# glaretechnologies/substrata

Hardware: AMD Instinct MI355X
Metric: physics steps/sec at fixed dt, 100k bodies (higher is better)
Workload: dtype f32; 1 GPU; BASELINE config 3: 100000 mixed box/sphere/capsule bodies, 100x100x10 lattice spacing 1.5 m, seed 3, ground quad 2000 m, dt 1/60, Jolt default settings (10 velocity / 2 position iterations), sleeping enabled; bodies_per_gpu=100000, tiles=1, active_bodies_end=99193, contact_constraints_start=296641, contact_constraints_end=299690, contact_points_end=362045, colours_end=21, contact_constraints_after_settle=293058, dropped_pairs_or_manifolds=0

## Files before the change

### substrata_amd/csrc/sgp_dev_common.h

```cpp
#pragma once
#include "sgp_kernels.h"
#include <algorithm>
#include "sgp_device_collide.h"
#include "sgp_device_vehicle.h"
#include "sgp_device_mesh.h"

#define TPB 256


SGP_DEV const ConstraintArrays& CUR(const DV& d) { return d.ca[d.sp->parity & 1]; }
SGP_DEV const ConstraintArrays& PRV(const DV& d) { return d.ca[(d.sp->parity & 1) ^ 1]; }
SGP_DEV uint2 con_ab(const ConstraintArrays& c, size_t k) { return *(const uint2*)(c.hdr + k); }
SGP_DEV int& con_npc(const ConstraintArrays& c, size_t k) { return ((int*)(c.hdr + k))[2]; }
SGP_DEV uint4 con_hdr(const ConstraintArrays& c, size_t k) { return c.hdr[k]; }

SGP_DEV uint32_t f_motion(uint32_t f) { return f & BF_MOTION_MASK; }
SGP_DEV uint32_t f_layer(uint32_t f) { return (f & BF_LAYER_MASK) >> BF_LAYER_SHIFT; }
SGP_DEV uint32_t f_shape(uint32_t f) { return (f & BF_SHAPE_MASK) >> BF_SHAPE_SHIFT; }
SGP_DEV bool f_movable(uint32_t f) { return (f & (BF_ALIVE | BF_ACTIVE)) == (BF_ALIVE | BF_ACTIVE) && f_motion(f) == SGP_MOTION_DYNAMIC; }
SGP_DEV uint32_t xcd_block() { return (blockIdx.x & 7u) * (gridDim.x >> 3) + (blockIdx.x >> 3); }
SGP_DEV bool f_active_for_pairs(uint32_t f) { return (f & (BF_ALIVE | BF_ACTIVE)) == (BF_ALIVE | BF_ACTIVE) && f_motion(f) != SGP_MOTION_STATIC; }

SGP_DEV bool layers_collide(uint32_t l1, uint32_t l2)
{
	if (l1 == SGP_LAYER_NON_MOVING) return l2 == SGP_LAYER_MOVING;
	if (l1 == SGP_LAYER_MOVING) return l2 != SGP_LAYER_NON_MOVING_NON_COLLIDABLE && l2 != SGP_LAYER_MOVING_NON_COLLIDABLE;
	return false;
}

SGP_DEV const sgd_hull* body_hull(const DV& d, float4 sh) { return &d.hulls[(uint32_t)sh.x]; }

SGP_DEV v3 shape_local_half(const DV& d, uint32_t type, float4 sh)
{
	if (type == SGP_SHAPE_MESH) return V3(1.0f, 1.0f, 1.0f);
	if (type == SGP_SHAPE_HULL) {
		const sgd_hull* h = body_hull(d, sh);
		return V3(fmaxf(fabsf(h->aabb_min.x), fabsf(h->aabb_max.x)), fmaxf(fabsf(h->aabb_min.y), fabsf(h->aabb_max.y)), fmaxf(fabsf(h->aabb_min.z), fabsf(h->aabb_max.z)));
	}
	if (type == SGP_SHAPE_SPHERE) return V3(sh.x, sh.x, sh.x);
	if (type == SGP_SHAPE_BOX) return V3(sh.x, sh.y, sh.z);
	return V3(sh.x, sh.x, sh.y + sh.x);
}

SGP_DEV float shape_volume(const DV& d, uint32_t type, float4 sh)
{
	if (type == SGP_SHAPE_MESH) return 0.0f;
	if (type == SGP_SHAPE_HULL) return body_hull(d, sh)->volume;
	if (type == SGP_SHAPE_SPHERE) return (4.0f / 3.0f) * 3.14159265358979323846f * sh.x * sh.x * sh.x;
	if (type == SGP_SHAPE_BOX) return 8.0f * sh.x * sh.y * sh.z;
	return 3.14159265358979323846f * sh.x * sh.x * (2.0f * sh.y) + (4.0f / 3.0f) * 3.14159265358979323846f * sh.x * sh.x * sh.x;
}

SGP_DEV void compute_aabb(const DV& d, uint32_t type, float4 sh, v3 pos, quat q, v3& mn, v3& mx)
{
	v3 e;
	if (type == SGP_SHAPE_MESH) {
		const MeshHeader mh = d.meshes[(uint32_t)sh.x];
		const m33 R = quat_to_m33(q);
		v3 lo = V3(3.4e38f, 3.4e38f, 3.4e38f), hi = V3(-3.4e38f, -3.4e38f, -3.4e38f);
		for (int k = 0; k < 8; ++k) {
			const v3 c = V3((k & 1) ? mh.mxx : mh.mnx, (k & 2) ? mh.mxy : mh.mny, (k & 4) ? mh.mxz : mh.mnz);
			const v3 p = m33_mul(R, c);
			lo = V3(fminf(lo.x, p.x), fminf(lo.y, p.y), fminf(lo.z, p.z)); hi = V3(fmaxf(hi.x, p.x), fmaxf(hi.y, p.y), fmaxf(hi.z, p.z));
		}
		mn = v3_add(pos, lo); mx = v3_add(pos, hi);
		return;
	}
	if (type == SGP_SHAPE_HULL) {
		const sgd_hull* h = body_hull(d, sh);
		const m33 R = quat_to_m33(q);
		v3 lo = V3(3.4e38f, 3.4e38f, 3.4e38f), hi = V3(-3.4e38f, -3.4e38f, -3.4e38f);
		for (int i = 0; i < h->nv; ++i) {
			const v3 p = m33_mul(R, h->verts[i]);
			lo = V3(fminf(lo.x, p.x), fminf(lo.y, p.y), fminf(lo.z, p.z)); hi = V3(fmaxf(hi.x, p.x), fmaxf(hi.y, p.y), fmaxf(hi.z, p.z));
		}
		mn = v3_add(pos, lo); mx = v3_add(pos, hi);
		return;
	}
	if (type == SGP_SHAPE_SPHERE) e = V3(sh.x, sh.x, sh.x);
	else {
		const m33 R = quat_to_m33(q);
		if (type == SGP_SHAPE_BOX) {
			e = V3(fabsf(R.c0.x) * sh.x + fabsf(R.c1.x) * sh.y + fabsf(R.c2.x) * sh.z,
			       fabsf(R.c0.y) * sh.x + fabsf(R.c1.y) * sh.y + fabsf(R.c2.y) * sh.z,
			       fabsf(R.c0.z) * sh.x + fabsf(R.c1.z) * sh.y + fabsf(R.c2.z) * sh.z);
		} else {
			e = V3(fabsf(R.c2.x) * sh.y + sh.x, fabsf(R.c2.y) * sh.y + sh.x, fabsf(R.c2.z) * sh.y + sh.x);
		}
	}
	mn = v3_sub(pos, e);
	mx = v3_add(pos, e);
}

SGP_DEV void sleep_points(const DV& d, uint32_t type, float4 sh, v3 pos, quat q, v3 out[3])
{
	const v3 ext = shape_local_half(d, type, sh);
	const m33 R = quat_to_m33(q);
	int lowest = 0;
	if (ext.y < v3_get(ext, lowest)) lowest = 1;
	if (ext.z < v3_get(ext, lowest)) lowest = 2;
	const int i1 = lowest == 0 ? 1 : 0;
	const int i2 = lowest == 2 ? 1 : 2;
	out[0] = pos;
	out[1] = v3_add(pos, v3_scale(m33_col(R, i1), v3_get(ext, i1)));
	out[2] = v3_add(pos, v3_scale(m33_col(R, i2), v3_get(ext, i2)));
}

SGP_DEV void reset_sleep(const DV& d, uint32_t i, uint32_t type, float4 sh, v3 pos, quat q)
{
	v3 p[3];
	sleep_points(d, type, sh, pos, q, p);
	d.sleep_s[0][i] = F4(p[0], 0.0f);
	d.sleep_s[1][i] = F4(p[1], 0.0f);
	d.sleep_s[2][i] = F4(p[2], 0.0f);
	d.sleep_timer[i] = 0.0f;
}

SGP_DEV void push_event(uint32_t* list, uint32_t* counter, uint32_t cap, uint32_t id)
{
	const uint32_t k = atomicAdd(counter, 1u);
	if (k < cap) list[k] = id;
}

SGP_DEV void step_end_block(const DV& d, StepCounters* host_mapped, EventWindow* host_events)
{
	const uint32_t* src = (const uint32_t*)d.ctr;
	uint32_t* dst = (uint32_t*)host_mapped;
	for (uint32_t i = threadIdx.x; i < sizeof(StepCounters) / 4; i += blockDim.x) dst[i] = src[i];
	__syncthreads();
	if (threadIdx.x == 0 && d.ts_nt) { host_mapped->ts_error = d.ts_flags[0]; host_mapped->ts_all_adjacent = d.ts_flags[1]; }
	if (threadIdx.x < sizeof(EventCounters) / 4) ((uint32_t*)&host_events->c)[threadIdx.x] = ((const uint32_t*)d.evc)[threadIdx.x];
	const uint32_t win = min(min(d.ev_window, SGP_EVENT_WINDOW), d.cap_bodies);
	const uint32_t* lists[3] = { d.ev_activated, d.ev_deactivated, d.ev_water };
	const uint32_t counts[3] = { d.evc->n_activated, d.evc->n_deactivated, d.evc->n_water };
	for (int l = 0; l < 3; ++l) {
		if (counts[l] > win) continue;
		for (uint32_t i = threadIdx.x; i < counts[l]; i += blockDim.x) host_events->ids[l][i] = lists[l][i];
	}
}

SGP_DEV bool last_block(uint32_t* ticket)
{
	__shared__ uint32_t s_last_ticket;
	__syncthreads();
	if (threadIdx.x == 0) { __threadfence(); s_last_ticket = atomicAdd(ticket, 1u); }
	__syncthreads();
	const bool last = s_last_ticket == gridDim.x - 1u;
	if (last) __threadfence();
	return last;
}

SGP_DEV int float_to_ordered(float f) { const int i = __float_as_int(f); return i >= 0 ? i : i ^ 0x7FFFFFFF; }
SGP_DEV float ordered_to_float(int i) { return __int_as_float(i >= 0 ? i : i ^ 0x7FFFFFFF); }


static inline uint32_t blocks_for(uint32_t n) { return n ? (n + TPB - 1) / TPB : 1; }
static inline uint32_t stride_grid(uint32_t estimate) { uint32_t b = blocks_for(estimate); if (b < 64) b = 64; if (b > 4096) b = 4096; return (b + 7u) & ~7u; }
```

### substrata_amd/csrc/sgp_dev_solve.h

```cpp
#pragma once

SGP_DEV sym33 body_world_inv_inertia(const DV& d, uint32_t body)
{
	return world_inv_inertia(quat_to_m33(Q4(d.pose[POSE_F4 * (size_t)body + 1])), V3(d.pose[POSE_F4 * (size_t)body + 2]));
}
SGP_DEV sym33 body_world_inv_inertia_rec(const DV& d, uint32_t body)
{
	const float4 a = d.vel[VEL_F4 * (size_t)body + 2], b = d.vel[VEL_F4 * (size_t)body + 3];
	sym33 s; s.xx = a.x; s.xy = a.y; s.xz = a.z; s.yy = a.w; s.yz = b.x; s.zz = b.y;
	return s;
}

SGP_DEV float lane_swap1(float x)
{
	return __int_as_float(__builtin_amdgcn_mov_dpp(__float_as_int(x), 0xB1, 0xF, 0xF, true));
}

struct ConHalf {
	uint32_t body;
	float4 nf; int np_col;
	v3     c[4][3];
	v3     iv[4][3];
	float  eff[4][3];
	float  bias[4];
	v3     t1;
	v3     lam[4];
};

template <int ROWS = -1> SGP_DEV void half_load_rows(const DV& d, uint32_t slot, int side, ConHalf& h)
{
	const int np = h.np_col & 0xFF;
	const size_t st = d.cap_manifolds;
	if (ROWS < 0 ? d.sp->compact_rows == 2u : ROWS == 2) {
		const sym33 I = body_world_inv_inertia_rec(d, h.body);
		const v3 n = V3(h.nf);
		h.t1 = v3_normalized_perpendicular(n);
		const v3 t2 = v3_cross(n, h.t1);
#pragma unroll
		for (int i = 0; i < 4; ++i) {
			if (i == 0 || i < np) {
				const float4 r4 = side ? CUR(d).r2e[i][slot] : CUR(d).r1b[i][slot];
				const float2 et = CUR(d).efft[i][slot];
				const v3 r = V3(r4);
				h.c[i][0] = v3_cross(r, n); h.c[i][1] = v3_cross(r, h.t1); h.c[i][2] = v3_cross(r, t2);
#pragma unroll
				for (int a = 0; a < 3; ++a) h.iv[i][a] = sym33_mul(I, h.c[i][a]);
				const float ow = lane_swap1(r4.w);
				h.eff[i][0] = side ? r4.w : ow; h.bias[i] = side ? ow : r4.w;
				h.eff[i][1] = et.x; h.eff[i][2] = et.y;
				h.lam[i] = V3(CUR(d).lam[i][slot]);
			}
		}
		return;
	}
	if (ROWS < 0 ? d.sp->compact_rows != 0u : ROWS != 0) {
		const sym33 I = body_world_inv_inertia_rec(d, h.body);
#pragma unroll
		for (int i = 0; i < 4; ++i) {
			if (i == 0 || i < np) {
#pragma unroll
				for (int a = 0; a < 3; ++a) {
					const float4 c4 = axis_rows(d, slot, i, a)[(size_t)side * st];
					h.c[i][a] = V3(c4); h.iv[i][a] = sym33_mul(I, V3(c4));
					const float ow = lane_swap1(c4.w);
					h.eff[i][a] = side ? c4.w : ow;
					if (a == 0) h.bias[i] = side ? ow : c4.w;
				}
				h.lam[i] = V3(CUR(d).lam[i][slot]);
			}
		}
		h.t1 = v3_normalized_perpendicular(V3(h.nf));
		return;
	}
#pragma unroll
	for (int i = 0; i < 4; ++i) {
		if (i == 0 || i < np) {
#pragma unroll
			for (int a = 0; a < 3; ++a) {
				const float4* p = axis_rows(d, slot, i, a);
				const float4 c4 = p[(size_t)side * st];
				const float4 i4 = p[(size_t)(2 + side) * st];
				h.c[i][a] = V3(c4); h.iv[i][a] = V3(i4);
				const float ow = lane_swap1(c4.w);
				h.eff[i][a] = side ? c4.w : ow;
				if (a == 0) h.bias[i] = side ? ow : c4.w;
				if (i == 0 && a < 2) {
					const float oi = lane_swap1(i4.w);
					if (a == 0) { h.t1.x = side ? oi : i4.w; h.t1.y = side ? i4.w : oi; } else h.t1.z = side ? oi : i4.w;
				}
			}
			const float4 l4 = CUR(d).lam[i][slot];
			h.lam[i] = V3(l4);
		}
	}
}

template <int ROWS = -1> SGP_DEV void half_load_known(const DV& d, uint32_t slot, int side, int np_col, uint32_t body, ConHalf& h)
{
	h.body = body;
	h.nf = CUR(d).n_fric[slot];
	h.np_col = np_col;
	half_load_rows<ROWS>(d, slot, side, h);
}
template <int ROWS = -1> SGP_DEV void half_load(const DV& d, uint32_t slot, int side, ConHalf& h)
{
	const uint4 hd = con_hdr(CUR(d), slot);
	half_load_known<ROWS>(d, slot, side, (int)hd.z, side ? hd.y : hd.x, h);
}

SGP_DEV void half_store(const DV& d, uint32_t slot, int side, const ConHalf& h)
{
	if (side) return;
	const int np = h.np_col & 0xFF;
#pragma unroll
	for (int i = 0; i < 4; ++i) { if (i < np) CUR(d).lam[i][slot] = F4(h.lam[i], 0.0f); }
}

SGP_DEV float half_jv(v3 lv, v3 av, v3 axis, v3 c, int side)
{
	const float mine = v3_dot(axis, lv) + v3_dot(c, av);
	const float other = lane_swap1(mine);
	return side ? other - mine : mine - other;
}
SGP_DEV void half_apply(v3& lv, v3& av, float im, v3 axis, v3 iv, float lambda, int side)
{
	if (!(im > 0.0f)) return;
	if (side) { lv = v3_add(lv, v3_scale(axis, lambda * im)); av = v3_add(av, v3_scale(iv, lambda)); }
	else      { lv = v3_sub(lv, v3_scale(axis, lambda * im)); av = v3_sub(av, v3_scale(iv, lambda)); }
}

SGP_DEV bool half_solve_core(ConHalf& h, int side, float4& v4, float4& w4, uint32_t dbg)
{
	const int np = h.np_col & 0xFF;
	const float im = v4.w, friction = h.nf.w;
	v3 lv = V3(v4), av = V3(w4);
	const v3 n = V3(h.nf);
	const v3 t1 = (dbg & 2u) ? v3_normalized_perpendicular(n) : h.t1;
	const v3 t2 = v3_cross(n, t1);
	if (friction > 0.0f) {
#pragma unroll
		for (int i = 0; i < 4; ++i) {
			if (i < np && !(h.eff[i][1] <= 0.0f && h.eff[i][2] <= 0.0f)) {
				float l1 = h.lam[i].y + h.eff[i][1] * half_jv(lv, av, t1, h.c[i][1], side);
				float l2 = h.lam[i].z + h.eff[i][2] * half_jv(lv, av, t2, h.c[i][2], side);
				const float max_f = friction * h.lam[i].x;
				const float tot_sq = l1 * l1 + l2 * l2;
				if (tot_sq > max_f * max_f) { const float sc = max_f / sqrtf(tot_sq); l1 = l1 * sc; l2 = l2 * sc; }
				half_apply(lv, av, im, t1, h.iv[i][1], l1 - h.lam[i].y, side); h.lam[i].y = l1;
				half_apply(lv, av, im, t2, h.iv[i][2], l2 - h.lam[i].z, side); h.lam[i].z = l2;
			}
		}
	}
#pragma unroll
	for (int i = 0; i < 4; ++i) {
		if (i < np && h.eff[i][0] > 0.0f) {
			const float jv = half_jv(lv, av, n, h.c[i][0], side);
			const float lambda = h.eff[i][0] * (jv - h.bias[i]);
			const float nl = max0f(h.lam[i].x + lambda);
			half_apply(lv, av, im, n, h.iv[i][0], nl - h.lam[i].x, side);
			h.lam[i].x = nl;
		}
	}
	v4 = F4(lv, im); w4 = F4(av, 0.0f);
	return im > 0.0f;
}
template <int VS> SGP_DEV void half_solve(ConHalf& h, int side, float4* vel, uint32_t dbg = 0)
{
	if ((h.np_col & 0xFF) == 0) return;
	float4 v4 = vel[VS * (size_t)h.body], w4 = vel[VS * (size_t)h.body + 1];
	if (half_solve_core(h, side, v4, w4, dbg)) { vel[VS * (size_t)h.body] = v4; vel[VS * (size_t)h.body + 1] = w4; }
}

template <int VS, int ROWS = -1> SGP_DEV void solve_velocity_pair_t(const DV& d, uint32_t slot, int side, float4* vel)
{
	ConHalf h;
	half_load<ROWS>(d, slot, side, h);
	half_solve<VS>(h, side, vel, d.dbg_flags);
	half_store(d, slot, side, h);
}

template <int VS> SGP_DEV void solve_velocity_pair_norows(const DV& d, uint32_t slot, int side, float4* vel)
{
	const uint4 hd = con_hdr(CUR(d), slot);
	const int np = (int)hd.z & 0xFF;
	const uint32_t body = side ? hd.y : hd.x;
	const float4 nf = CUR(d).n_fric[slot];
	float4 r4[4]; float2 et[4]; v3 lam[4];
#pragma unroll
	for (int i = 0; i < 4; ++i) {
		if (i == 0 || i < np) { r4[i] = side ? CUR(d).r2e[i][slot] : CUR(d).r1b[i][slot]; et[i] = CUR(d).efft[i][slot]; lam[i] = V3(CUR(d).lam[i][slot]); }
		else { r4[i] = make_float4(0.0f, 0.0f, 0.0f, 0.0f); et[i] = make_float2(0.0f, 0.0f); lam[i] = V3(0.0f, 0.0f, 0.0f); }
	}
	if (np == 0) return;
	const sym33 I = body_world_inv_inertia_rec(d, body);
	float4 v4 = vel[VS * (size_t)body], w4 = vel[VS * (size_t)body + 1];
	const float im = v4.w, friction = nf.w;
	v3 lv = V3(v4), av = V3(w4);
	const v3 n = V3(nf);
	const v3 t1 = v3_normalized_perpendicular(n);
	const v3 t2 = v3_cross(n, t1);
	float eff0[4], bias[4];
#pragma unroll
	for (int i = 0; i < 4; ++i) { const float ow = lane_swap1(r4[i].w); eff0[i] = side ? r4[i].w : ow; bias[i] = side ? ow : r4[i].w; }
	if (friction > 0.0f) {
#pragma unroll
		for (int i = 0; i < 4; ++i) {
			if (i < np && !(et[i].x <= 0.0f && et[i].y <= 0.0f)) {
				const v3 r = V3(r4[i]);
				const v3 c1 = v3_cross(r, t1), c2 = v3_cross(r, t2);
				float l1 = lam[i].y + et[i].x * half_jv(lv, av, t1, c1, side);
				float l2 = lam[i].z + et[i].y * half_jv(lv, av, t2, c2, side);
				const float max_f = friction * lam[i].x;
				const float tot_sq = l1 * l1 + l2 * l2;
				if (tot_sq > max_f * max_f) { const float sc = max_f / sqrtf(tot_sq); l1 = l1 * sc; l2 = l2 * sc; }
				half_apply(lv, av, im, t1, sym33_mul(I, c1), l1 - lam[i].y, side); lam[i].y = l1;
				half_apply(lv, av, im, t2, sym33_mul(I, c2), l2 - lam[i].z, side); lam[i].z = l2;
			}
		}
	}
#pragma unroll
	for (int i = 0; i < 4; ++i) {
		if (i < np && eff0[i] > 0.0f) {
			const v3 c0 = v3_cross(V3(r4[i]), n);
			const float jv = half_jv(lv, av, n, c0, side);
			const float lambda = eff0[i] * (jv - bias[i]);
			const float nl = max0f(lam[i].x + lambda);
			half_apply(lv, av, im, n, sym33_mul(I, c0), nl - lam[i].x, side);
			lam[i].x = nl;
		}
	}
	if (im > 0.0f) { vel[VS * (size_t)body] = F4(lv, im); vel[VS * (size_t)body + 1] = F4(av, 0.0f); }
	if (!side) {
#pragma unroll
		for (int i = 0; i < 4; ++i) { if (i < np) CUR(d).lam[i][slot] = F4(lam[i], 0.0f); }
	}
}

struct PosHalf { float4 nf; int np; v3 loc[4]; };
SGP_DEV void pos_half_load(const DV& d, uint32_t slot, int side, int np_col, PosHalf& ph)
{
	ph.nf = CUR(d).n_fric[slot];
	ph.np = np_col & 0xFF;
#pragma unroll
	for (int i = 0; i < 4; ++i) if (i == 0 || i < ph.np) ph.loc[i] = V3(side ? CUR(d).loc2[i][slot] : CUR(d).loc1[i][slot]);
}
SGP_DEV void pos_half_solve(const DV& d, const PosHalf& ph, int side, float4* rec, v3 ii)
{
	const v3 nrm = V3(ph.nf);
	const int np = ph.np;
	const float4 p4 = rec[0];
	const float im = p4.w;
	quat q = Q4(rec[1]);
	v3 pos = V3(p4);
	bool moved = false;
	m33 R = quat_to_m33(q);
#pragma unroll
	for (int i = 0; i < 4; ++i) {
		if (i >= np) continue;
		const v3 mine = v3_add(pos, m33_mul(R, ph.loc[i]));
		const v3 other = V3(lane_swap1(mine.x), lane_swap1(mine.y), lane_swap1(mine.z));
		const v3 p1 = side ? other : mine, p2 = side ? mine : other;
		float sep = v3_dot(v3_sub(p2, p1), nrm) + d.st.penetration_slop;
		if (sep < 0.0f) {
			sep = fmaxf(sep, -d.st.max_penetration_distance);
			const v3 mid = v3_scale(v3_add(p1, p2), 0.5f);
			const v3 r = v3_sub(mid, pos);
			v3 Ic = V3(0.0f, 0.0f, 0.0f);
			float share = 0.0f;
			if (im > 0.0f) { const v3 c = v3_cross(r, nrm); Ic = sym33_mul(world_inv_inertia(R, ii), c); share = im + v3_dot(Ic, c); }
			const float oshare = lane_swap1(share);
			const float s1 = side ? oshare : share, s2 = side ? share : oshare;
			const float inv = s1 + s2;
			const float eff = inv > 0.0f ? 1.0f / inv : 0.0f;
			if (eff <= 0.0f) continue;
			const float lambda = -eff * d.st.baumgarte * sep;
			if (im > 0.0f) {
				if (side) { pos = v3_add(pos, v3_scale(nrm, lambda * im)); q = quat_add_rotation_step(q, v3_scale(Ic, lambda)); }
				else      { pos = v3_sub(pos, v3_scale(nrm, lambda * im)); q = quat_add_rotation_step(q, v3_scale(Ic, -lambda)); }
				R = quat_to_m33(q);
			}
			moved = true;
		}
	}
	if (moved && im > 0.0f) { rec[0] = F4(pos, im); rec[1] = make_float4(q.x, q.y, q.z, q.w); }
}
SGP_DEV void solve_position_pair(const DV& d, uint32_t slot, int side)
{
	const uint4 hd = con_hdr(CUR(d), slot);
	const uint32_t body = side ? hd.y : hd.x;
	PosHalf ph;
	pos_half_load(d, slot, side, (int)hd.z, ph);
	pos_half_solve(d, ph, side, d.pose + POSE_F4 * (size_t)body, V3(d.pose[POSE_F4 * (size_t)body + 2]));
}
SGP_DEV void solve_position_pair_at(const DV& d, uint32_t slot, int side, float4* rec, v3 ii)
{
	PosHalf ph;
	pos_half_load(d, slot, side, con_npc(CUR(d), slot), ph);
	pos_half_solve(d, ph, side, rec, ii);
}
#define SOLVE_VEL_TPB 256
#define SOLVE_XCD_CHUNKS 0x100

SGP_DEV uint32_t uf_prio(uint32_t x);
SGP_DEV uint32_t uf_find(const uint32_t* parent, uint32_t x);
```

### substrata_amd/csrc/sgp_k_solve.hip

```cpp
#include "sgp_dev_all.h"


struct BodyVel { v3 lv, av; };

SGP_DEV void apply_impulse(BodyVel& A, BodyVel& B, float im1, const sym33& I1, float im2, const sym33& I2, v3 r1, v3 r2, v3 axis, float lambda)
{
	if (im1 > 0.0f) {
		A.lv = v3_sub(A.lv, v3_scale(axis, lambda * im1));
		A.av = v3_sub(A.av, v3_scale(sym33_mul(I1, v3_cross(r1, axis)), lambda));
	}
	if (im2 > 0.0f) {
		B.lv = v3_add(B.lv, v3_scale(axis, lambda * im2));
		B.av = v3_add(B.av, v3_scale(sym33_mul(I2, v3_cross(r2, axis)), lambda));
	}
}

SGP_DEV float axis_jv(const BodyVel& A, const BodyVel& B, v3 r1, v3 r2, v3 axis)
{
	return (v3_dot(axis, A.lv) + v3_dot(v3_cross(r1, axis), A.av)) - (v3_dot(axis, B.lv) + v3_dot(v3_cross(r2, axis), B.av));
}

struct PairCtx { uint2 ab; float im1, im2; sym33 I1, I2; BodyVel A, B; v3 n, t1, t2; float friction; int np; };
template <int VS> SGP_DEV void load_pair(const DV& d, uint32_t slot, PairCtx& c, const float4* vel)
{
	const uint4 hd = con_hdr(CUR(d), slot);
	c.ab = make_uint2(hd.x, hd.y);
	const float4 nf = CUR(d).n_fric[slot];
	c.n = V3(nf); c.friction = nf.w;
	c.np = (int)hd.z & 0xFF;
	const float4 va = vel[VS * (size_t)c.ab.x], wa = vel[VS * (size_t)c.ab.x + 1];
	const float4 vb = vel[VS * (size_t)c.ab.y], wb = vel[VS * (size_t)c.ab.y + 1];
	c.im1 = va.w; c.im2 = vb.w;
	c.I1 = c.im1 > 0.0f ? body_world_inv_inertia(d, c.ab.x) : sym33_zero();
	c.I2 = c.im2 > 0.0f ? body_world_inv_inertia(d, c.ab.y) : sym33_zero();
	c.A.lv = V3(va); c.A.av = V3(wa);
	c.B.lv = V3(vb); c.B.av = V3(wb);
}

template <int VS> SGP_DEV void store_pair_vel(const PairCtx& c, float4* vel)
{
	if (c.im1 > 0.0f) { vel[VS * (size_t)c.ab.x] = F4(c.A.lv, c.im1); vel[VS * (size_t)c.ab.x + 1] = F4(c.A.av, 0.0f); }
	if (c.im2 > 0.0f) { vel[VS * (size_t)c.ab.y] = F4(c.B.lv, c.im2); vel[VS * (size_t)c.ab.y + 1] = F4(c.B.av, 0.0f); }
}

template <int VS> SGP_DEV void warm_start_one_t(const DV& d, uint32_t slot, float4* vel)
{
	PairCtx c;
	load_pair<VS>(d, slot, c, vel);
	c.t1 = v3_normalized_perpendicular(c.n);
	c.t2 = v3_cross(c.n, c.t1);
	v3 P = V3(0.0f, 0.0f, 0.0f), A1 = V3(0.0f, 0.0f, 0.0f), A2 = V3(0.0f, 0.0f, 0.0f);
#pragma unroll
	for (int i = 0; i < 4; ++i) {
		if (i < c.np) {
			const v3 r1 = V3(CUR(d).r1b[i][slot]), r2 = V3(CUR(d).r2e[i][slot]);
			const float4 l = CUR(d).lam[i][slot];
			v3 j = v3_scale(c.n, l.x);
			if (c.friction > 0.0f) { j = v3_add(j, v3_scale(c.t1, l.y)); j = v3_add(j, v3_scale(c.t2, l.z)); }
			P = v3_add(P, j);
			A1 = v3_add(A1, v3_cross(r1, j));
			A2 = v3_add(A2, v3_cross(r2, j));
		}
	}
	if (c.im1 > 0.0f) { c.A.lv = v3_add(c.A.lv, v3_neg(v3_scale(P, c.im1))); c.A.av = v3_add(c.A.av, v3_neg(sym33_mul(c.I1, A1))); }
	if (c.im2 > 0.0f) { c.B.lv = v3_add(c.B.lv, v3_scale(P, c.im2)); c.B.av = v3_add(c.B.av, sym33_mul(c.I2, A2)); }
	store_pair_vel<VS>(c, vel);
}
SGP_DEV void warm_start_one(const DV& d, uint32_t slot) { warm_start_one_t<VEL_F4>(d, slot, d.vel); }

SGP_DEV void warm_body_one(const DV& d, uint32_t i)
{
	if (i >= d.sp->n_slots) return;
	uint64_t mask = d.colour_mask[i] & ~(1ull << SGP_OVERFLOW_COLOUR);
	if (!mask) return;
	float4* rec = d.vel + VEL_F4 * (size_t)i;
	const float4 v4 = rec[0], w4 = rec[1];
	const float im = v4.w;
	if (!(im > 0.0f)) return;
	const float4* wr = d.warm + (size_t)i * SGP_MAX_COLOURS * 2;
	v3 lv = V3(v4), av = V3(w4);
	while (mask) {
		int col[4]; float4 a[4], b[4];
#pragma unroll
		for (int k = 0; k < 4; ++k) {
			col[k] = mask ? __ffsll((long long)mask) - 1 : -1;
			if (mask) mask &= mask - 1;
			if (col[k] >= 0) { a[k] = wr[2 * col[k]]; b[k] = wr[2 * col[k] + 1]; }
		}
#pragma unroll
		for (int k = 0; k < 4; ++k) if (col[k] >= 0) { lv = v3_add(lv, V3(a[k])); av = v3_add(av, V3(b[k])); }
	}
	rec[0] = F4(lv, im);
	rec[1] = F4(av, 0.0f);
}
SGP_DEV void warm_start_one(const DV& d, uint32_t k);
SGP_DEV uint32_t overflow_next(const DV& d, uint32_t first, uint32_t count, uint64_t& last, bool& have_last);
__global__ void __launch_bounds__(TPB) k_warm_bodies(DV d)
{
	warm_body_one(d, blockIdx.x * TPB + threadIdx.x);
	const uint32_t first = d.cstarts[SGP_OVERFLOW_COLOUR], count = d.cstarts[SGP_OVERFLOW_COLOUR + 1] - first;
	if (count == 0u) return;
	if (!last_block(&d.ctr->tickets[1]) || threadIdx.x != 0) return;
	uint64_t last = 0; bool have_last = false;
	for (uint32_t it = 0; it < count; ++it) warm_start_one(d, overflow_next(d, first, count, last, have_last));
}
struct AxisRows { float4 c1, c2, i1, i2; };

SGP_DEV AxisRows load_axis_rows(const DV& d, uint32_t slot, int point, int axis)
{
	const float4* p = axis_rows(d, slot, point, axis);
	const size_t st = d.cap_manifolds;
	AxisRows r; r.c1 = p[0]; r.c2 = p[st]; r.i1 = p[2 * st]; r.i2 = p[3 * st];
	return r;
}

SGP_DEV float rows_jv(const BodyVel& A, const BodyVel& B, v3 axis, const AxisRows& r)
{
	return (v3_dot(axis, A.lv) + v3_dot(V3(r.c1), A.av)) - (v3_dot(axis, B.lv) + v3_dot(V3(r.c2), B.av));
}

SGP_DEV void rows_apply(BodyVel& A, BodyVel& B, float im1, float im2, v3 axis, const AxisRows& r, float lambda)
{
	if (im1 > 0.0f) {
		A.lv = v3_sub(A.lv, v3_scale(axis, lambda * im1));
		A.av = v3_sub(A.av, v3_scale(V3(r.i1), lambda));
	}
	if (im2 > 0.0f) {
		B.lv = v3_add(B.lv, v3_scale(axis, lambda * im2));
		B.av = v3_add(B.av, v3_scale(V3(r.i2), lambda));
	}
}

SGP_DEV void solve_position_one(const DV& d, uint32_t slot)
{
	const uint4 hd = con_hdr(CUR(d), slot);
	const uint2 ab = make_uint2(hd.x, hd.y);
	const float4 nf = CUR(d).n_fric[slot];
	const v3 nrm = V3(nf);
	const int np = (int)hd.z & 0xFF;
	float4* ra = d.pose + POSE_F4 * (size_t)ab.x;
	float4* rb = d.pose + POSE_F4 * (size_t)ab.y;
	const float4 pa = ra[0], pb = rb[0];
	const float im1 = pa.w, im2 = pb.w;
	quat qa = Q4(ra[1]), qb = Q4(rb[1]);
	const v3 iiA = V3(d.pose[POSE_F4 * (size_t)ab.x + 2]), iiB = V3(d.pose[POSE_F4 * (size_t)ab.y + 2]);
	v3 posA = V3(pa), posB = V3(pb);
	bool moved = false;
	m33 RA = quat_to_m33(qa), RB = quat_to_m33(qb);
#pragma unroll
	for (int i = 0; i < 4; ++i) {
		if (i >= np) continue;
		const v3 p1 = v3_add(posA, m33_mul(RA, V3(CUR(d).loc1[i][slot])));
		const v3 p2 = v3_add(posB, m33_mul(RB, V3(CUR(d).loc2[i][slot])));
		float sep = v3_dot(v3_sub(p2, p1), nrm) + d.st.penetration_slop;
		if (sep < 0.0f) {
			sep = fmaxf(sep, -d.st.max_penetration_distance);
			const v3 mid = v3_scale(v3_add(p1, p2), 0.5f);
			const v3 r1 = v3_sub(mid, posA), r2 = v3_sub(mid, posB);
			sym33 I1 = sym33_zero(), I2 = sym33_zero();
			if (im1 > 0.0f) I1 = world_inv_inertia(RA, iiA);
			if (im2 > 0.0f) I2 = world_inv_inertia(RB, iiB);
			const float eff = axis_eff_mass(im1, I1, r1, im2, I2, r2, nrm);
			if (eff <= 0.0f) continue;
			const float lambda = -eff * d.st.baumgarte * sep;
			if (im1 > 0.0f) {
				posA = v3_sub(posA, v3_scale(nrm, lambda * im1));
				qa = quat_add_rotation_step(qa, v3_scale(sym33_mul(I1, v3_cross(r1, nrm)), -lambda));
				RA = quat_to_m33(qa);
			}
			if (im2 > 0.0f) {
				posB = v3_add(posB, v3_scale(nrm, lambda * im2));
				qb = quat_add_rotation_step(qb, v3_scale(sym33_mul(I2, v3_cross(r2, nrm)), lambda));
				RB = quat_to_m33(qb);
			}
			moved = true;
		}
	}
	if (moved) {
		if (im1 > 0.0f) { ra[0] = F4(posA, pa.w); ra[1] = make_float4(qa.x, qa.y, qa.z, qa.w); }
		if (im2 > 0.0f) { rb[0] = F4(posB, pb.w); rb[1] = make_float4(qb.x, qb.y, qb.z, qb.w); }
	}
}

#define SOLVE_TPB 64
template <int MODE, int ROWS = -1, int OCC = 1> __global__ void __launch_bounds__(MODE != 0 ? SOLVE_VEL_TPB : SOLVE_TPB, OCC) k_solve_colour(const uint32_t* cstarts_pre, StepParams* sp_pre, DV d_arg, int colour_arg)
{
	DV d = d_arg; d.sp = sp_pre;
	const int colour = colour_arg & 0xFF;
	const uint32_t first = cstarts_pre[colour], end = cstarts_pre[colour + 1];
	if (MODE != 0) {
		const int side = (int)(threadIdx.x & 1u);
		const uint32_t bx = (colour_arg & SOLVE_XCD_CHUNKS) ? xcd_block() : blockIdx.x;
		for (uint32_t k = first + ((bx * SOLVE_VEL_TPB + threadIdx.x) >> 1); k < end; k += gridDim.x * (SOLVE_VEL_TPB / 2)) {
			if (MODE == 1) { if constexpr (ROWS == 2) solve_velocity_pair_norows<VEL_F4>(d, k, side, d.vel); else solve_velocity_pair_t<VEL_F4, ROWS>(d, k, side, d.vel); }
			else solve_position_pair(d, k, side);
		}
		return;
	}
	for (uint32_t k = first + blockIdx.x * SOLVE_TPB + threadIdx.x; k < end; k += gridDim.x * SOLVE_TPB) warm_start_one(d, k);
}


SGP_DEV uint32_t overflow_next(const DV& d, uint32_t first, uint32_t count, uint64_t& last, bool& have_last)
{
	uint64_t best = ~0ull; uint32_t bslot = first;
	for (uint32_t k = 0; k < count; ++k) {
		const uint2 okab = con_ab(CUR(d), first + k); const uint64_t pr = sgp_mix64(((uint64_t)okab.x << 32) | okab.y);
		if ((!have_last || pr > last) && pr <= best) { best = pr; bslot = first + k; }
	}
	last = best; have_last = true;
	return bslot;
}

__global__ void __launch_bounds__(512) k_solve_tail(DV d, int first_colour, int mode)
{
	__shared__ uint32_t cs[SGP_MAX_COLOURS + 1];
	if (threadIdx.x <= SGP_MAX_COLOURS) cs[threadIdx.x] = d.cstarts[threadIdx.x];
	__syncthreads();
	if (cs[first_colour] == cs[SGP_MAX_COLOURS]) return;
	for (int c = first_colour; c < SGP_OVERFLOW_COLOUR; ++c) {
		const uint32_t b = cs[c], e = cs[c + 1];
		if (b == e) continue;
		for (uint32_t k = b + threadIdx.x; k < e; k += 512) {
			if (mode == 0) warm_start_one(d, k); else solve_position_one(d, k);
		}
		__syncthreads();
	}
	const uint32_t first = cs[SGP_OVERFLOW_COLOUR], count = cs[SGP_OVERFLOW_COLOUR + 1] - first;
	if (count == 0 || threadIdx.x != 0) return;
	uint64_t last = 0; bool have_last = false;
	for (uint32_t it = 0; it < count; ++it) {
		const uint32_t bslot = overflow_next(d, first, count, last, have_last);
		if (mode == 0) warm_start_one(d, bslot); else solve_position_one(d, bslot);
	}
}

#define TAIL_VEL_TPB 768
template <int ROWS> __global__ void __launch_bounds__(TAIL_VEL_TPB) k_solve_tail_vel(DV d, int first_colour)
{
	__shared__ uint32_t cs[SGP_MAX_COLOURS + 1];
	if (threadIdx.x <= SGP_MAX_COLOURS) cs[threadIdx.x] = d.cstarts[threadIdx.x];
	__syncthreads();
	if (cs[first_colour] == cs[SGP_MAX_COLOURS]) return;
	const int side = (int)(threadIdx.x & 1u);
	const uint32_t pair = threadIdx.x >> 1;
	const uint32_t tail_n = cs[SGP_OVERFLOW_COLOUR] - cs[first_colour];
	if (tail_n <= TAIL_VEL_TPB / 2 && !(d.dbg_flags & 1u)) {
		const uint32_t slot = cs[first_colour] + pair;
		const bool mine = pair < tail_n;
		ConHalf h; int my_col = -1;
		if (mine) { half_load<ROWS>(d, slot, side, h); my_col = (h.np_col >> 8) & 0xFF; }
		for (int c = first_colour; c < SGP_OVERFLOW_COLOUR; ++c) {
			if (cs[c] == cs[c + 1]) continue;
			if (my_col == c) half_solve<VEL_F4>(h, side, d.vel, d.dbg_flags);
			__syncthreads();
		}
		if (mine) half_store(d, slot, side, h);
	} else
	for (int c = first_colour; c < SGP_OVERFLOW_COLOUR; ++c) {
		const uint32_t b = cs[c], e = cs[c + 1];
		if (b == e) continue;
		for (uint32_t k = b + pair; k < e; k += TAIL_VEL_TPB / 2) solve_velocity_pair_t<VEL_F4, ROWS>(d, k, side, d.vel);
		__syncthreads();
	}
	const uint32_t first = cs[SGP_OVERFLOW_COLOUR], count = cs[SGP_OVERFLOW_COLOUR + 1] - first;
	if (count == 0 || threadIdx.x >= 2) return;
	uint64_t last = 0; bool have_last = false;
	for (uint32_t it = 0; it < count; ++it) {
		const uint32_t bslot = overflow_next(d, first, count, last, have_last);
		solve_velocity_pair_t<VEL_F4, ROWS>(d, bslot, side, d.vel);
	}
}
#define HC_CLASSES 9
#define HC_WG_PAIRS 256
#define HC_TPB (2 * HC_WG_PAIRS)
#define HC_BIG 0xFFFFFFFFu
#define HC_NONE 0xFFFFFFFFu
#define NPCOL_CATCH_ALL (1 << 17)
#define HC_BIG_LIST (4 * HC_WG_PAIRS)

SGP_DEV bool hc_can_move(const DV& d, uint32_t body) { return d.vel[VEL_F4 * (size_t)body].w > 0.0f; }

__global__ void __launch_bounds__(TPB) k_hc_hook(DV d, int first_colour)
{
	const uint32_t b = d.cstarts[first_colour], e = d.cstarts[SGP_OVERFLOW_COLOUR];
	const uint32_t tid = blockIdx.x * TPB + threadIdx.x, stride = gridDim.x * TPB;
	const uint32_t lim = min(2u * (e - b) + HC_CLASSES * HC_WG_PAIRS, d.cap_hc_list);
	for (uint32_t i = tid; i < lim; i += stride) d.hc_list[i] = HC_NONE;
	for (uint32_t k = b + tid; k < e; k += stride) {
		const uint2 ab = con_ab(CUR(d), k);
		if (!hc_can_move(d, ab.x) || !hc_can_move(d, ab.y)) continue;
		uint32_t ra = uf_find(d.hc_root, ab.x), rb = uf_find(d.hc_root, ab.y);
		while (ra != rb) {
			const bool a_hi = uf_prio(ra) > uf_prio(rb);
			const uint32_t hi = a_hi ? ra : rb, lo = a_hi ? rb : ra;
			const uint32_t old = atomicCAS(&d.hc_root[hi], hi, lo);
			if (old == hi) break;
			ra = uf_find(d.hc_root, old); rb = uf_find(d.hc_root, lo);
		}
	}
}
SGP_DEV uint32_t hc_root_of(const DV& d, uint2 ab)
{
	const uint32_t x = hc_can_move(d, ab.x) ? ab.x : (hc_can_move(d, ab.y) ? ab.y : HC_NONE);
	return x == HC_NONE ? HC_NONE : uf_find(d.hc_root, x);
}
__global__ void __launch_bounds__(TPB) k_hc_count(DV d, int first_colour)
{
	const uint32_t b = d.cstarts[first_colour], e = d.cstarts[SGP_OVERFLOW_COLOUR];
	for (uint32_t k = b + blockIdx.x * TPB + threadIdx.x; k < e; k += gridDim.x * TPB) {
		const uint32_t r = hc_root_of(d, con_ab(CUR(d), k));
		d.hc_rank[k] = r == HC_NONE ? 0u : atomicAdd(&d.hc_count[r], 1u);
	}
}
__global__ void __launch_bounds__(TPB) k_hc_alloc(DV d, int first_colour)
{
	const uint32_t b = d.cstarts[first_colour], e = d.cstarts[SGP_OVERFLOW_COLOUR];
	const int lane = (int)(threadIdx.x & 63u);
	for (uint32_t k0 = b + blockIdx.x * TPB; k0 < e; k0 += gridDim.x * TPB) {
		const uint32_t k = k0 + threadIdx.x;
		uint32_t r = HC_NONE, size = 0;
		if (k < e && d.hc_rank[k] == 0u) { r = hc_root_of(d, con_ab(CUR(d), k)); if (r != HC_NONE) size = d.hc_count[r]; }
		const bool lead = r != HC_NONE;
		int cls = -1;
		if (lead) {
			if (size > (uint32_t)HC_WG_PAIRS) d.hc_base[r] = HC_BIG;
			else cls = size <= 1u ? 0 : 32 - __clz((int)(size - 1u));
		}
		unsigned long long mine_m = 0ull;
#pragma unroll
		for (int c = 0; c < HC_CLASSES; ++c) { const unsigned long long m = __ballot(cls == c); if (cls == c) mine_m = m; }
		const int leader = mine_m ? __ffsll((long long)mine_m) - 1 : lane;
		uint32_t base = 0;
		if (cls >= 0 && lane == leader) base = atomicAdd(&d.ctr->hc_class[cls], (uint32_t)__popcll(mine_m));
		base = __shfl(base, leader, 64);
		if (cls >= 0) d.hc_base[r] = ((uint32_t)cls << 28) | (base + (uint32_t)__popcll(mine_m & ((1ull << lane) - 1ull)));
	}
}
SGP_DEV uint32_t hc_class_first(const DV& d, int cls)
{
	uint32_t first = 0;
	for (int c = 0; c < cls; ++c) first += ((d.ctr->hc_class[c] << c) + (HC_WG_PAIRS - 1)) & ~(uint32_t)(HC_WG_PAIRS - 1);
	return first;
}
__global__ void __launch_bounds__(TPB) k_hc_scatter(DV d, int first_colour)
{
	const uint32_t b = d.cstarts[first_colour], e = d.cstarts[SGP_OVERFLOW_COLOUR];
	if (blockIdx.x == 0 && threadIdx.x == 0) { d.ctr->hc_entries = hc_class_first(d, HC_CLASSES); d.ctr->hc_n = e - b; }
	for (uint32_t k = b + blockIdx.x * TPB + threadIdx.x; k < e; k += gridDim.x * TPB) {
		const uint32_t r = hc_root_of(d, con_ab(CUR(d), k));
		const uint32_t place = r == HC_NONE ? HC_BIG : d.hc_base[r];
		uint32_t at = HC_NONE;
		if (place != HC_BIG) {
			const int cls = (int)(place >> 28);
			at = hc_class_first(d, cls) + ((place & 0x0FFFFFFFu) << cls) + d.hc_rank[k];
		}
		if (at < d.cap_hc_list) d.hc_list[at] = k;
		else {
			con_npc(CUR(d), k) |= NPCOL_CATCH_ALL;
			const uint32_t bi = wave_alloc(&d.ctr->hc_n_big);
			if (bi < HC_BIG_LIST) d.hc_big_list[bi] = k;
		}
	}
}

__global__ void __launch_bounds__(TPB) k_hc_init(DV d, int first_colour)
{
	const uint32_t b = d.cstarts[first_colour], e = d.cstarts[SGP_OVERFLOW_COLOUR];
	for (uint32_t k = b + blockIdx.x * TPB + threadIdx.x; k < e; k += gridDim.x * TPB) {
		const uint2 ab = con_ab(CUR(d), k);
		if (hc_can_move(d, ab.x)) { d.hc_root[ab.x] = ab.x; d.hc_count[ab.x] = 0u; }
		if (hc_can_move(d, ab.y)) { d.hc_root[ab.y] = ab.y; d.hc_count[ab.y] = 0u; }
	}
}
__global__ void __launch_bounds__(TPB) k_hc_probe(DV d, int first_colour)
{
	const uint32_t b = d.cstarts[first_colour], e = d.cstarts[SGP_OVERFLOW_COLOUR];
	for (uint32_t k = b + blockIdx.x * TPB + threadIdx.x; k < e; k += gridDim.x * TPB) {
		if (d.hc_rank[k] != 0u) continue;
		const uint32_t r = hc_root_of(d, con_ab(CUR(d), k));
		if (r == HC_NONE) continue;
		const uint32_t size = d.hc_count[r];
		if (size > (uint32_t)HC_WG_PAIRS) atomicAdd(&d.ctr->hc_probe_big, size);
	}
}

__global__ void __launch_bounds__(HC_WG_PAIRS) k_hc_sort(DV d)
{
	__shared__ uint32_t s_cnt[SGP_MAX_COLOURS], s_first[SGP_MAX_COLOURS];
	__shared__ uint4 s_slot[HC_WG_PAIRS];
	const uint32_t entries = d.ctr->hc_entries;
	for (uint32_t e0 = blockIdx.x * HC_WG_PAIRS; e0 < entries; e0 += gridDim.x * HC_WG_PAIRS) {
		if (threadIdx.x < SGP_MAX_COLOURS) s_cnt[threadIdx.x] = 0u;
		__syncthreads();
		const uint32_t slot = d.hc_list[e0 + threadIdx.x];
		const uint4 hd = slot != HC_NONE ? con_hdr(CUR(d), slot) : make_uint4(0u, 0u, 0u, 0u);
		const int npc = (int)hd.z;
		const uint2 ab = make_uint2(hd.x, hd.y);
		const int col = slot != HC_NONE ? ((npc >> 8) & 0xFF) : SGP_MAX_COLOURS - 1;
		const uint32_t rank = atomicAdd(&s_cnt[col], 1u);
		__syncthreads();
		if (threadIdx.x < 64) {
			const uint32_t v = s_cnt[threadIdx.x];
			uint32_t x = v;
			for (int off = 1; off < 64; off <<= 1) { const uint32_t y = __shfl_up(x, off, 64); if ((int)threadIdx.x >= off) x += y; }
			s_first[threadIdx.x] = x - v;
		}
		__syncthreads();
		s_slot[s_first[col] + rank] = make_uint4(slot, (uint32_t)npc, ab.x, ab.y);
		__syncthreads();
		d.hc_entry[e0 + threadIdx.x] = s_slot[threadIdx.x];
		__syncthreads();
	}
}

#define HC_TABLE 1024
template <int MODE, int ROWS = -1> __global__ void __launch_bounds__(HC_TPB) k_solve_hc(const StepCounters* ctr_pre, const uint4* hc_entry_pre, DV d, int first_colour)
{
	constexpr int RS = MODE == 1 ? 2 : 3;
	__shared__ float4 s_rec[HC_TABLE * RS];
	__shared__ uint32_t s_key[HC_TABLE];
	__shared__ unsigned long long s_present;
	__shared__ uint32_t s_ticket;
	const int side = (int)(threadIdx.x & 1u);
	const uint32_t pair = threadIdx.x >> 1;
	const uint32_t entries = ctr_pre->hc_entries;
	const int n_colours = (int)ctr_pre->n_colours;
	for (uint32_t e0 = blockIdx.x * HC_WG_PAIRS; e0 < entries; e0 += gridDim.x * HC_WG_PAIRS) {
		__syncthreads();
		for (uint32_t i = threadIdx.x; i < HC_TABLE; i += HC_TPB) s_key[i] = HC_NONE;
		if (threadIdx.x == 0) s_present = 0ull;
		__syncthreads();
		const uint4 entry = hc_entry_pre[e0 + pair];
		const uint32_t slot = entry.x;
		const bool mine = slot != HC_NONE;
		ConHalf h; PosHalf ph; int my_col = -1;
		uint32_t body = HC_NONE, at = 0; bool owner = false;
		if (mine) {
			my_col = ((int)entry.y >> 8) & 0xFF;
			body = side ? entry.w : entry.z;
			if (MODE == 1) half_load_known<ROWS>(d, slot, side, (int)entry.y, body, h); else pos_half_load(d, slot, side, (int)entry.y, ph);
			if (side == 0) atomicOr(&s_present, 1ull << my_col);
			at = uf_prio(body) & (HC_TABLE - 1);
			for (;;) {
				const uint32_t old = atomicCAS(&s_key[at], HC_NONE, body);
				if (old == HC_NONE) { owner = true; break; }
				if (old == body) break;
				at = (at + 1) & (HC_TABLE - 1);
			}
			if (owner) {
				const float4* g = (MODE == 1 ? d.vel + VEL_F4 * (size_t)body : d.pose + POSE_F4 * (size_t)body);
				s_rec[RS * at] = g[0]; s_rec[RS * at + 1] = g[1];
				if (MODE != 1) s_rec[RS * at + 2] = d.pose[POSE_F4 * (size_t)body + 2];
			}
			if (MODE == 1) h.body = at;
		}
		__syncthreads();
		const unsigned long long present = s_present;
		for (int c = first_colour; c < n_colours; ++c) {
			if (!((present >> c) & 1ull)) continue;
			if (my_col == c) { if (MODE == 1) half_solve<2>(h, side, s_rec, d.dbg_flags); else pos_half_solve(d, ph, side, s_rec + RS * at, V3(s_rec[RS * at + 2])); }
			__syncthreads();
		}
		if (MODE == 1 && mine) half_store(d, slot, side, h);
		if (owner && s_rec[RS * at].w > 0.0f) {
			float4* g = (MODE == 1 ? d.vel + VEL_F4 * (size_t)body : d.pose + POSE_F4 * (size_t)body);
			g[0] = s_rec[RS * at]; g[1] = s_rec[RS * at + 1];
		}
	}
	const uint32_t n_big = d.ctr->hc_n_big;
	const uint32_t ofirst = d.cstarts[SGP_OVERFLOW_COLOUR], ocount = d.cstarts[SGP_OVERFLOW_COLOUR + 1] - ofirst;
	if (n_big == 0u && ocount == 0u) return;
	__syncthreads();
	if (threadIdx.x == 0) { __threadfence(); s_ticket = atomicAdd(&d.ctr->hc_done, 1u); }
	__syncthreads();
	if (s_ticket != gridDim.x - 1u) return;
	if (threadIdx.x == 0) d.ctr->hc_done = 0u;
	__threadfence();
	if (n_big != 0u && n_big <= (uint32_t)HC_BIG_LIST) {
		uint32_t mine[4]; int mcol[4]; int cnt = 0;
		for (uint32_t e = pair; e < n_big; e += HC_WG_PAIRS) { const uint32_t k = d.hc_big_list[e]; mine[cnt] = k; mcol[cnt] = (int)((con_npc(CUR(d), k) >> 8) & 0xFF); ++cnt; }
		for (int c = first_colour; c < n_colours; ++c) {
#pragma unroll
			for (int j = 0; j < 4; ++j) if (j < cnt && mcol[j] == c) { if (MODE == 1) solve_velocity_pair_t<VEL_F4, ROWS>(d, mine[j], side, d.vel); else solve_position_pair(d, mine[j], side); }
			__syncthreads();
		}
	} else
	for (int c = first_colour; c < n_colours && n_big != 0u; ++c) {
		const uint32_t cb = d.cstarts[c], ce = d.cstarts[c + 1];
		for (uint32_t k = cb + pair; k < ce; k += HC_WG_PAIRS) {
			if (!(con_npc(CUR(d), k) & NPCOL_CATCH_ALL)) continue;
			if (MODE == 1) solve_velocity_pair_t<VEL_F4, ROWS>(d, k, side, d.vel); else solve_position_pair(d, k, side);
		}
		__syncthreads();
	}
	if (ocount == 0u || threadIdx.x >= 2u) return;
	uint64_t last = 0; bool have_last = false;
	for (uint32_t it = 0; it < ocount; ++it) {
		const uint32_t bslot = overflow_next(d, ofirst, ocount, last, have_last);
		if (MODE == 1) solve_velocity_pair_t<VEL_F4, ROWS>(d, bslot, side, d.vel); else solve_position_pair(d, bslot, side);
	}
}

#define SMALL_LDS_BODIES 2048
#define SMALL_TPB 768
__global__ void __launch_bounds__(SMALL_TPB) k_solve_small(DV d, int warm_start, int iterations)
{
	__shared__ float4 sv[2 * SMALL_LDS_BODIES];
	__shared__ uint32_t cs[SGP_MAX_COLOURS + 1];
	const uint32_t n = min(d.sp->n_slots, (uint32_t)SMALL_LDS_BODIES);
	if (threadIdx.x <= SGP_MAX_COLOURS) cs[threadIdx.x] = d.cstarts[threadIdx.x];
	for (uint32_t i = threadIdx.x; i < 2 * n; i += SMALL_TPB) sv[i] = d.vel[VEL_F4 * (size_t)(i >> 1) + (i & 1u)];
	__syncthreads();
	const int side = (int)(threadIdx.x & 1u);
	const uint32_t pair = threadIdx.x >> 1;
	const uint32_t all_n = cs[SGP_OVERFLOW_COLOUR];
	if (all_n != 0 && all_n <= SMALL_TPB / 2 && cs[SGP_OVERFLOW_COLOUR] == cs[SGP_MAX_COLOURS]) {
		const uint32_t slot = pair;
		const bool mine = slot < all_n;
		if (warm_start) {
			for (int c = 0; c < SGP_OVERFLOW_COLOUR; ++c) {
				const uint32_t b = cs[c], e = cs[c + 1];
				if (b == e) continue;
				if (side == 0 && slot >= b && slot < e) warm_start_one_t<2>(d, slot, sv);
				__syncthreads();
			}
		}
		ConHalf h; int my_col = -1;
		if (mine) { half_load<0>(d, slot, side, h); my_col = (h.np_col >> 8) & 0xFF; }
		for (int pass = 0; pass < iterations; ++pass) {
			for (int c = 0; c < SGP_OVERFLOW_COLOUR; ++c) {
				if (cs[c] == cs[c + 1]) continue;
				if (my_col == c) half_solve<2>(h, side, sv, d.dbg_flags);
				__syncthreads();
			}
		}
		if (mine) half_store(d, slot, side, h);
	} else
	if (cs[0] != cs[SGP_MAX_COLOURS]) {
		for (int pass = warm_start ? -1 : 0; pass < iterations; ++pass) {
			for (int c = 0; c < SGP_OVERFLOW_COLOUR; ++c) {
				const uint32_t b = cs[c], e = cs[c + 1];
				if (b == e) continue;
				if (pass < 0) { for (uint32_t k = b + threadIdx.x; k < e; k += SMALL_TPB) warm_start_one_t<2>(d, k, sv); }
				else { for (uint32_t k = b + pair; k < e; k += SMALL_TPB / 2) solve_velocity_pair_t<2, 0>(d, k, side, sv); }
				__syncthreads();
			}
			const uint32_t first = cs[SGP_OVERFLOW_COLOUR], count = cs[SGP_OVERFLOW_COLOUR + 1] - first;
			if (count != 0) {
				if (threadIdx.x < 2) {
					uint64_t last = 0; bool have_last = false;
					for (uint32_t it = 0; it < count; ++it) {
						const uint32_t bslot = overflow_next(d, first, count, last, have_last);
						if (pass < 0) { if (side == 0) warm_start_one_t<2>(d, bslot, sv); } else solve_velocity_pair_t<2, 0>(d, bslot, side, sv);
					}
				}
				__syncthreads();
			}
		}
	}
	for (uint32_t i = threadIdx.x; i < 2 * n; i += SMALL_TPB) d.vel[VEL_F4 * (size_t)(i >> 1) + (i & 1u)] = sv[i];
}

struct ConReg { uint2 ab; float4 nf; int np_col; AxisRows rn[4], rt1[4], rt2[4]; float4 lam[4]; };

SGP_DEV void con_load(const DV& d, uint32_t slot, ConReg& r)
{
	const uint4 hd = con_hdr(CUR(d), slot);
	r.ab = make_uint2(hd.x, hd.y);
	r.nf = CUR(d).n_fric[slot];
	r.np_col = (int)hd.z;
	const int np = r.np_col & 0xFF;
#pragma unroll
	for (int i = 0; i < 4; ++i) {
		if (i < np) {
			r.rn[i] = load_axis_rows(d, slot, i, 0); r.rt1[i] = load_axis_rows(d, slot, i, 1); r.rt2[i] = load_axis_rows(d, slot, i, 2);
			r.lam[i] = CUR(d).lam[i][slot];
		}
	}
}

SGP_DEV void con_store(const DV& d, uint32_t slot, const ConReg& r)
{
	const int np = r.np_col & 0xFF;
#pragma unroll
	for (int i = 0; i < 4; ++i) { if (i < np) CUR(d).lam[i][slot] = r.lam[i]; }
}

template <int VS> SGP_DEV void con_solve_velocity(ConReg& r, float4* vel, uint32_t dbg = 0)
{
	const uint2 ab = r.ab;
	const int np = r.np_col & 0xFF;
	if (np == 0) return;
	const float4 va = vel[VS * (size_t)ab.x], wa = vel[VS * (size_t)ab.x + 1];
	const float4 vb = vel[VS * (size_t)ab.y], wb = vel[VS * (size_t)ab.y + 1];
	const float im1 = va.w, im2 = vb.w, friction = r.nf.w;
	BodyVel A, B;
	A.lv = V3(va); A.av = V3(wa); B.lv = V3(vb); B.av = V3(wb);
	const v3 n = V3(r.nf);
	const v3 t1 = (dbg & 2u) ? v3_normalized_perpendicular(n) : V3(r.rn[0].i1.w, r.rn[0].i2.w, r.rt1[0].i1.w);
	const v3 t2 = v3_cross(n, t1);
	if (friction > 0.0f) {
#pragma unroll
		for (int i = 0; i < 4; ++i) {
			if (i < np && !(r.rt1[i].c2.w <= 0.0f && r.rt2[i].c2.w <= 0.0f)) {
				float l1 = r.lam[i].y + r.rt1[i].c2.w * rows_jv(A, B, t1, r.rt1[i]);
				float l2 = r.lam[i].z + r.rt2[i].c2.w * rows_jv(A, B, t2, r.rt2[i]);
				const float max_f = friction * r.lam[i].x;
				const float tot_sq = l1 * l1 + l2 * l2;
				if (tot_sq > max_f * max_f) { const float sc = max_f / sqrtf(tot_sq); l1 = l1 * sc; l2 = l2 * sc; }
				rows_apply(A, B, im1, im2, t1, r.rt1[i], l1 - r.lam[i].y); r.lam[i].y = l1;
				rows_apply(A, B, im1, im2, t2, r.rt2[i], l2 - r.lam[i].z); r.lam[i].z = l2;
			}
		}
	}
#pragma unroll
	for (int i = 0; i < 4; ++i) {
		if (i < np && r.rn[i].c2.w > 0.0f) {
			const float jv = rows_jv(A, B, n, r.rn[i]);
			const float lambda = r.rn[i].c2.w * (jv - r.rn[i].c1.w);
			const float nl = max0f(r.lam[i].x + lambda);
			rows_apply(A, B, im1, im2, n, r.rn[i], nl - r.lam[i].x);
			r.lam[i].x = nl;
		}
	}
	if (im1 > 0.0f) { vel[VS * (size_t)ab.x] = F4(A.lv, im1); vel[VS * (size_t)ab.x + 1] = F4(A.av, 0.0f); }
	if (im2 > 0.0f) { vel[VS * (size_t)ab.y] = F4(B.lv, im2); vel[VS * (size_t)ab.y + 1] = F4(B.av, 0.0f); }
}

template <int VS> SGP_DEV void solve_velocity_one_t(const DV& d, uint32_t slot, float4* vel)
{
	ConReg r;
	con_load(d, slot, r);
	con_solve_velocity<VS>(r, vel, d.dbg_flags);
	con_store(d, slot, r);
}
__global__ void __launch_bounds__(512) k_solve_small_single(DV d, int warm_start, int iterations)
{
	__shared__ float4 sv[2 * SMALL_LDS_BODIES];
	__shared__ uint32_t cs[SGP_MAX_COLOURS + 1];
	const uint32_t n = min(d.sp->n_slots, (uint32_t)SMALL_LDS_BODIES);
	if (threadIdx.x <= SGP_MAX_COLOURS) cs[threadIdx.x] = d.cstarts[threadIdx.x];
	for (uint32_t i = threadIdx.x; i < 2 * n; i += 512) sv[i] = d.vel[VEL_F4 * (size_t)(i >> 1) + (i & 1u)];
	__syncthreads();
	const uint32_t all_n = cs[SGP_OVERFLOW_COLOUR];
	if (all_n != 0 && all_n <= 512u && cs[SGP_OVERFLOW_COLOUR] == cs[SGP_MAX_COLOURS]) {
		const uint32_t slot = threadIdx.x;
		const bool mine = slot < all_n;
		if (warm_start) {
			for (int c = 0; c < SGP_OVERFLOW_COLOUR; ++c) {
				const uint32_t b = cs[c], e = cs[c + 1];
				if (b == e) continue;
				if (slot >= b && slot < e) warm_start_one_t<2>(d, slot, sv);
				__syncthreads();
			}
		}
		ConReg r; int my_col = -1;
		if (mine) { con_load(d, slot, r); my_col = (r.np_col >> 8) & 0xFF; }
		for (int pass = 0; pass < iterations; ++pass) {
			for (int c = 0; c < SGP_OVERFLOW_COLOUR; ++c) {
				if (cs[c] == cs[c + 1]) continue;
				if (my_col == c) con_solve_velocity<2>(r, sv, d.dbg_flags);
				__syncthreads();
			}
		}
		if (mine) con_store(d, slot, r);
	} else
	if (cs[0] != cs[SGP_MAX_COLOURS]) {
		for (int pass = warm_start ? -1 : 0; pass < iterations; ++pass) {
			for (int c = 0; c < SGP_OVERFLOW_COLOUR; ++c) {
				const uint32_t b = cs[c], e = cs[c + 1];
				if (b == e) continue;
				for (uint32_t k = b + threadIdx.x; k < e; k += 512) {
					if (pass < 0) warm_start_one_t<2>(d, k, sv); else solve_velocity_one_t<2>(d, k, sv);
				}
				__syncthreads();
			}
			const uint32_t first = cs[SGP_OVERFLOW_COLOUR], count = cs[SGP_OVERFLOW_COLOUR + 1] - first;
			if (count != 0) {
				if (threadIdx.x == 0) {
					uint64_t last = 0; bool have_last = false;
					for (uint32_t it = 0; it < count; ++it) {
						uint64_t best = ~0ull; uint32_t bslot = first;
						for (uint32_t k = 0; k < count; ++k) {
							const uint2 okab = con_ab(CUR(d), first + k); const uint64_t pr = sgp_mix64(((uint64_t)okab.x << 32) | okab.y);
							if ((!have_last || pr > last) && pr <= best) { best = pr; bslot = first + k; }
						}
						last = best; have_last = true;
						if (pass < 0) warm_start_one_t<2>(d, bslot, sv); else solve_velocity_one_t<2>(d, bslot, sv);
					}
				}
				__syncthreads();
			}
		}
	}
	for (uint32_t i = threadIdx.x; i < 2 * n; i += 512) d.vel[VEL_F4 * (size_t)(i >> 1) + (i & 1u)] = sv[i];
}
#ifndef SGP_EXPERIMENTS
void launch_solve_probe(const DV&, int, int, uint32_t, hipStream_t) {}
void launch_ts_label(const DV&, uint32_t, hipStream_t) {}
void launch_colour_count_ts(const DV&, uint32_t, hipStream_t) {}
void launch_setup_ts(const DV&, uint32_t, hipStream_t) {}
void launch_ts_solve(const DV&, int, int, hipStream_t) {}
#endif
#define SOLVE_MANY_MIN 131072u
#ifndef SOLVE_MANY_OCC
#define SOLVE_MANY_OCC 3
#endif
void launch_solve_colour(const DV& d, int colour, uint32_t est, int mode, hipStream_t s, int compact_rows)
{
	uint32_t blocks = (est + est / 8 + 64 + SOLVE_TPB - 1) / SOLVE_TPB;
	if (mode != 0) blocks = (est + est / 8 + 64 + SOLVE_VEL_TPB / 2 - 1) / (SOLVE_VEL_TPB / 2);
	if (blocks > 8192) blocks = 8192;
	if (mode != 0) blocks = (blocks + 7u) & ~7u;
	if (mode != 0 && est >= 8192u && est <= 65536u) colour |= SOLVE_XCD_CHUNKS;
	if (mode == 0) hipLaunchKernelGGL(k_solve_colour<0>, dim3(blocks), dim3(SOLVE_TPB), 0, s, (const uint32_t*)d.cstarts, d.sp, d, colour);
	else if (mode == 1) {
		const bool many = est > SOLVE_MANY_MIN;
		if (compact_rows == 2) hipLaunchKernelGGL((k_solve_colour<1, 2>), dim3(blocks), dim3(SOLVE_VEL_TPB), 0, s, (const uint32_t*)d.cstarts, d.sp, d, colour);
		else if (compact_rows) { if (many) hipLaunchKernelGGL((k_solve_colour<1, 1, SOLVE_MANY_OCC>), dim3(blocks), dim3(SOLVE_VEL_TPB), 0, s, (const uint32_t*)d.cstarts, d.sp, d, colour); else hipLaunchKernelGGL((k_solve_colour<1, 1>), dim3(blocks), dim3(SOLVE_VEL_TPB), 0, s, (const uint32_t*)d.cstarts, d.sp, d, colour); }
		else hipLaunchKernelGGL((k_solve_colour<1, 0>), dim3(blocks), dim3(SOLVE_VEL_TPB), 0, s, (const uint32_t*)d.cstarts, d.sp, d, colour);
	}
	else if (est > SOLVE_MANY_MIN) hipLaunchKernelGGL((k_solve_colour<2, -1, SOLVE_MANY_OCC>), dim3(blocks), dim3(SOLVE_VEL_TPB), 0, s, (const uint32_t*)d.cstarts, d.sp, d, colour);
	else hipLaunchKernelGGL(k_solve_colour<2>, dim3(blocks), dim3(SOLVE_VEL_TPB), 0, s, (const uint32_t*)d.cstarts, d.sp, d, colour);
}
void launch_warm_bodies(const DV& d, uint32_t nb, hipStream_t s) { hipLaunchKernelGGL(k_warm_bodies, dim3(blocks_for(nb)), dim3(TPB), 0, s, d); }
void launch_solve_tail(const DV& d, int first_colour, int mode, hipStream_t s, int compact_rows)
{
	if (mode == 1) {
		if (compact_rows == 2) hipLaunchKernelGGL(k_solve_tail_vel<2>, dim3(1), dim3(TAIL_VEL_TPB), 0, s, d, first_colour);
		else if (compact_rows) hipLaunchKernelGGL(k_solve_tail_vel<1>, dim3(1), dim3(TAIL_VEL_TPB), 0, s, d, first_colour);
		else hipLaunchKernelGGL(k_solve_tail_vel<0>, dim3(1), dim3(TAIL_VEL_TPB), 0, s, d, first_colour);
	}
	else hipLaunchKernelGGL(k_solve_tail, dim3(1), dim3(512), 0, s, d, first_colour, mode);
}
void launch_hc_build(const DV& d, int first_colour, uint32_t est, hipStream_t s)
{
	const uint32_t blocks = std::max(1u, std::min(1024u, (est + est / 8 + TPB - 1) / TPB));
	hipLaunchKernelGGL(k_hc_hook, dim3(blocks), dim3(TPB), 0, s, d, first_colour);
	hipLaunchKernelGGL(k_hc_count, dim3(blocks), dim3(TPB), 0, s, d, first_colour);
	hipLaunchKernelGGL(k_hc_alloc, dim3(blocks), dim3(TPB), 0, s, d, first_colour);
	hipLaunchKernelGGL(k_hc_scatter, dim3(blocks), dim3(TPB), 0, s, d, first_colour);
	hipLaunchKernelGGL(k_hc_sort, dim3(std::max(1u, std::min(2048u, (2u * est + HC_CLASSES * HC_WG_PAIRS) / HC_WG_PAIRS))), dim3(HC_WG_PAIRS), 0, s, d);
}
void launch_hc_probe(const DV& d, int probe_colour, uint32_t probe_est, hipStream_t s)
{
	const uint32_t pb = std::max(1u, std::min(1024u, (probe_est + probe_est / 8 + TPB - 1) / TPB));
	hipLaunchKernelGGL(k_hc_hook, dim3(pb), dim3(TPB), 0, s, d, probe_colour);
	hipLaunchKernelGGL(k_hc_count, dim3(pb), dim3(TPB), 0, s, d, probe_colour);
	hipLaunchKernelGGL(k_hc_probe, dim3(pb), dim3(TPB), 0, s, d, probe_colour);
	hipLaunchKernelGGL(k_hc_init, dim3(pb), dim3(TPB), 0, s, d, probe_colour);
}
void launch_solve_hc(const DV& d, int first_colour, uint32_t est, int mode, hipStream_t s, int compact_rows)
{
	const uint32_t blocks = std::max(1u, std::min(2048u, (2u * est + HC_CLASSES * HC_WG_PAIRS) / HC_WG_PAIRS));
	if (mode == 1) {
		if (compact_rows == 2) hipLaunchKernelGGL((k_solve_hc<1, 2>), dim3(blocks), dim3(HC_TPB), 0, s, (const StepCounters*)d.ctr, (const uint4*)d.hc_entry, d, first_colour);
		else if (compact_rows) hipLaunchKernelGGL((k_solve_hc<1, 1>), dim3(blocks), dim3(HC_TPB), 0, s, (const StepCounters*)d.ctr, (const uint4*)d.hc_entry, d, first_colour);
		else hipLaunchKernelGGL((k_solve_hc<1, 0>), dim3(blocks), dim3(HC_TPB), 0, s, (const StepCounters*)d.ctr, (const uint4*)d.hc_entry, d, first_colour);
	}
	else hipLaunchKernelGGL((k_solve_hc<2, -1>), dim3(blocks), dim3(HC_TPB), 0, s, (const StepCounters*)d.ctr, (const uint4*)d.hc_entry, d, first_colour);
}
void launch_solve_small(const DV& d, int warm_start, int iterations, int lane_pairs, hipStream_t s)
{
	if (lane_pairs) hipLaunchKernelGGL(k_solve_small, dim3(1), dim3(SMALL_TPB), 0, s, d, warm_start, iterations);
	else hipLaunchKernelGGL(k_solve_small_single, dim3(1), dim3(512), 0, s, d, warm_start, iterations);
}
```

### substrata_amd/csrc/sgp_k_vehicle.hip

```cpp
#include "sgp_dev_all.h"

template <bool CYL> SGP_DEV void veh_cast_test(const DV& d, const sgd_vehicle* v, v3 o, v3 dir, float rs, float cast_len, uint32_t j, float& best, uint32_t& bid, v3& bn, v3& bp, const sgd_wheel* wh = nullptr)
{
	if (j == v->body) return;
	const uint32_t f = d.flags[j];
	if (!(f & BF_ALIVE) || (f & (BF_SENSOR | BF_ALIAS))) return;
	const uint32_t layer = f_layer(f);
	if (!(layer == SGP_LAYER_NON_MOVING || layer == SGP_LAYER_MOVING)) return;
	const float4 mn = d.aabb_min[j], mx = d.aabb_max[j];
	const float e = rs + 1.0e-3f;
	if (!ray_aabb(o, dir, make_float4(mn.x - e, mn.y - e, mn.z - e, 0.0f), make_float4(mx.x + e, mx.y + e, mx.z + e, 0.0f), cast_len)) return;
	const float4 sh = d.pose[POSE_F4 * (size_t)j + 3];
	const float prm[3] = { sh.x, sh.y, sh.z };
	v3 n, p;
	float t;
	if (CYL && wh) {
		t = f_shape(f) == SGP_SHAPE_MESH ? cast_disc_mesh(d, j, o, dir, wh->cast_e, wh->cast_din, wh->disc_r, wh->cast_rho, cast_len, &n, &p)
		  : sgd_cast_disc_body((int)f_shape(f), prm, f_shape(f) == SGP_SHAPE_HULL ? body_hull(d, sh) : nullptr, V3(d.pose[POSE_F4 * (size_t)j]), quat_to_m33(Q4(d.pose[POSE_F4 * (size_t)j + 1])), o, dir, wh->cast_e, wh->cast_din, wh->disc_r, wh->cast_rho, cast_len, &n, &p);
		if (t > best) t = -1.0f;
	} else
	t = f_shape(f) == SGP_SHAPE_MESH ? cast_sphere_mesh(d, j, o, dir, best, rs, &n, &p)
	  : sgd_cast_sphere_body((int)f_shape(f), prm, f_shape(f) == SGP_SHAPE_HULL ? body_hull(d, sh) : nullptr, V3(d.pose[POSE_F4 * (size_t)j]), quat_to_m33(Q4(d.pose[POSE_F4 * (size_t)j + 1])), o, dir, best, rs, &n, &p);
	if (t < 0.0f || (!(CYL && wh) && n.z < v->cos_max_slope)) return;
	if (t < best || bid == SGP_INVALID_ID || (t == best && j < bid)) { best = t; bid = j; bn = n; bp = p; }
}

SGP_DEV sgd_chassis veh_chassis_pose_vel(const DV& d, uint32_t b)
{
	sgd_chassis c;
	const float4 p = d.pose[POSE_F4 * (size_t)b];
	c.pos = V3(p); c.rot = Q4(d.pose[POSE_F4 * (size_t)b + 1]); c.v = V3(d.vel[VEL_F4 * (size_t)b]); c.w = V3(d.vel[VEL_F4 * (size_t)b + 1]);
	c.im = p.w; c.inv_inertia_local = V3(d.pose[POSE_F4 * (size_t)b + 2]);
	c.I = world_inv_inertia(quat_to_m33(c.rot), c.inv_inertia_local);
	return c;
}

SGP_DEV void veh_stage_in(sgd_vehicle* sv, const sgd_vehicle* gv)
{
	const uint32_t* src = (const uint32_t*)gv; uint32_t* dst = (uint32_t*)sv;
	for (uint32_t i = threadIdx.x; i < sizeof(sgd_vehicle) / 4; i += 64) dst[i] = src[i];
	__syncthreads();
}
SGP_DEV void veh_stage_out(sgd_vehicle* gv, const sgd_vehicle* sv)
{
	__syncthreads();
	const uint32_t* src = (const uint32_t*)sv; uint32_t* dst = (uint32_t*)gv;
	for (uint32_t i = threadIdx.x; i < sizeof(sgd_vehicle) / 4; i += 64) dst[i] = src[i];
}

template <bool CYL> __global__ void __launch_bounds__(64) k_vehicle_cast(DV d)
{
	__shared__ sgd_vehicle sv;
	__shared__ int s_dormant;
	const uint32_t k = blockIdx.x;
	sgd_vehicle* gv = &d.vehicles[k];
	if ((k & 31u) == 0u && threadIdx.x == 0) d.veh_defer_bits[k >> 5] = 0u;
	if (!gv->alive) return;
	veh_stage_in(&sv, gv);
	if (threadIdx.x == 0) {
		const sgp_vehicle_input in = d.vehicle_inputs[k];
		sv.in_forward = in.forward; sv.in_right = in.right; sv.in_brake = in.brake; sv.in_handbrake = in.hand_brake;
		const uint32_t b = sv.body;
		const uint32_t fb = b < d.sp->n_slots ? d.flags[b] : 0u;
		sv.active = f_movable(fb) ? 1 : 0;
		s_dormant = (!sv.active && (fb & BF_ALIVE) && !(fb & BF_ACTIVE) && f_motion(fb) == SGP_MOTION_DYNAMIC) ? 1 : 0;
	}
	__syncthreads();
	const bool dormant = s_dormant != 0;
	if (sv.active || dormant) {
		{ const sgd_chassis c = veh_chassis_pose_vel(d, sv.body); sgd_vehicle_precast_lanes(&sv, &c, d.sp->dt, (int)threadIdx.x); }
		__syncthreads();
		const int wi = (int)(threadIdx.x >> 4); const uint32_t sub = threadIdx.x & 15u;
		float best = 0.0f; uint32_t bid = SGP_INVALID_ID; v3 bn = V3(0.0f, 0.0f, 0.0f), bp = bn;
		if (wi < sv.num_wheels) {
			const sgd_wheel* wh = &sv.wheels[wi];
			const v3 o = wh->cast_origin, dir = wh->cast_dir;
			const bool cyl = CYL && sv.tester == SGP_VEHICLE_TESTER_CYLINDER;
			const float rs = cyl ? wh->radius : sv.cast_radius;
			const sgd_wheel* const whc = cyl ? wh : nullptr;
			best = wh->cast_len;
			for (uint32_t l = sub; l < d.sp->n_large; l += 16) veh_cast_test<CYL>(d, &sv, o, dir, rs, wh->cast_len, d.large_ids[l], best, bid, bn, bp, whc);
			{
				const v3 e2 = v3_add(o, v3_scale(dir, wh->cast_len));
				const float m2 = rs + 2.0e-3f;
				uint32_t seen = 0;
				large_grid_query(d, V3(fminf(o.x, e2.x) - m2, fminf(o.y, e2.y) - m2, fminf(o.z, e2.z) - m2), V3(fmaxf(o.x, e2.x) + m2, fmaxf(o.y, e2.y) + m2, fmaxf(o.z, e2.z) + m2),
				                 [&](uint32_t i) { if ((seen++ & 15u) == sub) veh_cast_test<CYL>(d, &sv, o, dir, rs, wh->cast_len, i, best, bid, bn, bp, whc); });
			}
			const BpGrid g = *d.grid;
			if (g.n_cells > 0 && g.min_x <= g.max_x) {
				const v3 e = v3_add(o, v3_scale(dir, wh->cast_len));
				const float m = rs + 1.0e-3f;
				const int x0 = max((int)floorf((fminf(o.x, e.x) - m - g.ox) * g.inv_cell) - 1, 0), x1 = min((int)floorf((fmaxf(o.x, e.x) + m - g.ox) * g.inv_cell) + 1, g.nx - 1);
				const int y0 = max((int)floorf((fminf(o.y, e.y) - m - g.oy) * g.inv_cell) - 1, 0), y1 = min((int)floorf((fmaxf(o.y, e.y) + m - g.oy) * g.inv_cell) + 1, g.ny - 1);
				const int z0 = max((int)floorf((fminf(o.z, e.z) - m - g.oz) * g.inv_cell) - 1, 0), z1 = min((int)floorf((fmaxf(o.z, e.z) + m - g.oz) * g.inv_cell) + 1, g.nz - 1);
				if (x0 <= x1) for (int z = z0; z <= z1; ++z) for (int y = y0; y <= y1; ++y) {
					grid_row_runs(d, g, x0, x1, y, z, [&](uint32_t q0, uint32_t q1) { for (uint32_t q = q0 + sub; q < q1; q += 16) veh_cast_test<CYL>(d, &sv, o, dir, rs, wh->cast_len, __float_as_uint(d.sorted_max[q].w), best, bid, bn, bp, whc); });
				}
			}
		}
#pragma unroll
		for (int off = 8; off >= 1; off >>= 1) {
			const float ot = __shfl_xor(best, off, 16); const uint32_t oid = __shfl_xor(bid, off, 16);
			const float onx = __shfl_xor(bn.x, off, 16), ony = __shfl_xor(bn.y, off, 16), onz = __shfl_xor(bn.z, off, 16);
			const float opx = __shfl_xor(bp.x, off, 16), opy = __shfl_xor(bp.y, off, 16), opz = __shfl_xor(bp.z, off, 16);
			const bool take = oid != SGP_INVALID_ID && (bid == SGP_INVALID_ID || ot < best || (ot == best && oid < bid));
			if (take) { best = ot; bid = oid; bn = V3(onx, ony, onz); bp = V3(opx, opy, opz); }
		}
		if (dormant) {
			const bool hit = wi < sv.num_wheels && sub == 0 && bid != SGP_INVALID_ID;
			const uint32_t fh = hit ? d.flags[bid] : 0u;
			if (__ballot(hit && (fh & BF_ACTIVE) && f_motion(fh) != SGP_MOTION_STATIC) == 0ull) {
				if (threadIdx.x == 0) gv->active = 0;
				return;
			}
			if (threadIdx.x == 0) { sv.active = 1; wake_body(d, sv.body); }
		}
		if (wi < sv.num_wheels && sub == 0 && bid != SGP_INVALID_ID) {
			const uint32_t fo = d.flags[bid];
			v3 gvel = V3(0.0f, 0.0f, 0.0f);
			if (f_motion(fo) != SGP_MOTION_STATIC) gvel = v3_add(V3(d.vel[VEL_F4 * (size_t)bid]), v3_cross(V3(d.vel[VEL_F4 * (size_t)bid + 1]), v3_sub(bp, V3(d.pose[POSE_F4 * (size_t)bid]))));
			sgd_vehicle_set_hit(&sv, wi, bid, best, bn, bp, gvel, d.pose[POSE_F4 * (size_t)bid + 3].w);
			if (f_motion(fo) == SGP_MOTION_DYNAMIC) {
				sv.wheels[wi].ground_dynamic = 1;
				if (!(fo & BF_ACTIVE)) wake_body(d, bid);
				atomicMax((unsigned long long*)&d.veh_claim[bid], ((unsigned long long)*d.veh_epoch << 32) | (unsigned long long)(0xFFFFFFFFu - k));
			}
		}
		if (threadIdx.x == 0) atomicMax((unsigned long long*)&d.veh_claim[sv.body], ((unsigned long long)*d.veh_epoch << 32) | (unsigned long long)(0xFFFFFFFFu - k));
	}
	veh_stage_out(gv, &sv);
}

SGP_DEV void veh_export(const DV& d, uint32_t k, const sgd_vehicle& v, int deferred);
__global__ void __launch_bounds__(64) k_vehicle_controller(DV d)
{
	__shared__ sgd_vehicle sv;
	int sv_deferred = 0;
	sgd_vehicle* gv = &d.vehicles[blockIdx.x];
	if (!gv->alive || !gv->active) { if (threadIdx.x == 0) d.veh_head[(size_t)blockIdx.x * VEH_HEAD_F4] = make_float4(0.0f, 0.0f, 0.0f, 0.0f); return; }
	veh_stage_in(&sv, gv);
	{
		const uint32_t b = sv.body;
		sgd_chassis c = veh_chassis_pose_vel(d, b);
		const float lvw = d.vel[VEL_F4 * (size_t)b].w, avw = d.vel[VEL_F4 * (size_t)b + 1].w;
		sgd_ground g; g.dyn = 0; g.pos = V3(0.0f, 0.0f, 0.0f); g.im = 0.0f; g.I = sym33_zero();
		bool lost = false;
		const unsigned long long my_claim = ((unsigned long long)*d.veh_epoch << 32) | (unsigned long long)(0xFFFFFFFFu - blockIdx.x);
		if ((int)threadIdx.x < sv.num_wheels && sv.wheels[threadIdx.x].has_contact && sv.wheels[threadIdx.x].ground_dynamic) {
			const uint32_t gb = sv.wheels[threadIdx.x].contact_body;
			const float4 gp = d.pose[POSE_F4 * (size_t)gb];
			g.dyn = 1; g.pos = V3(gp); g.im = gp.w;
			g.I = world_inv_inertia(quat_to_m33(Q4(d.pose[POSE_F4 * (size_t)gb + 1])), V3(d.pose[POSE_F4 * (size_t)gb + 2]));
			lost = d.veh_claim[gb] != my_claim;
		}
		if (threadIdx.x == 0 && d.veh_claim[b] != my_claim) lost = true;
		if (__any(lost)) { sv_deferred = 1; if (threadIdx.x == 0) { atomicOr(&d.veh_defer_bits[blockIdx.x >> 5], 1u << (blockIdx.x & 31u)); atomicAdd(&d.ctr->veh_deferred, 1u); } }
		const int spinning = sgd_vehicle_controller_lanes(&sv, &c, &g, d.sp->dt, (int)threadIdx.x);
		if (threadIdx.x == 0) {
			if (spinning) d.sleep_timer[b] = 0.0f;
			d.vel[VEL_F4 * (size_t)b] = F4(c.v, lvw); d.vel[VEL_F4 * (size_t)b + 1] = F4(c.w, avw);
		}
	}
	__syncthreads();
	veh_export(d, blockIdx.x, sv, sv_deferred);
	veh_stage_out(gv, &sv);
}

#define VEH_CHUNK_LONG 1
#define VEH_CHUNK_LAT 2
#define VEH_CHUNK_GVEL 3
#define VEH_CHUNK_CPOS 4
#define VEH_CHUNK_MISC 5
#define VEH_CHUNK_ROW 6
#define VEH_CHUNK_WPOS 14
#define VEH_CHUNK_SDIR 15

template <int I> SGP_DEV float quad_bcast(float x) { return __int_as_float(__builtin_amdgcn_mov_dpp(__float_as_int(x), I * 0x55, 0xF, 0xF, true)); }
template <int I> SGP_DEV v3 quad_bcast(v3 a) { return V3(quad_bcast<I>(a.x), quad_bcast<I>(a.y), quad_bcast<I>(a.z)); }

SGP_DEV float4 veh_export_chunk(const sgd_vehicle& v, int i, int c)
{
	const sgd_wheel& w = v.wheels[i];
	const sgd_axis_part* part[4] = { &w.suspension, &w.max_up, &w.longitudinal, &w.lateral };
	if (i >= v.num_wheels) return make_float4(0.0f, 0.0f, 0.0f, 0.0f);
	if (c == VEH_CHUNK_NORMAL) return F4(w.contact_normal, __uint_as_float((w.has_contact ? 1u : 0u) | (w.suspension.active ? 2u : 0u) | (w.max_up.active ? 4u : 0u) | (w.longitudinal.active ? 8u : 0u) | (w.lateral.active ? 16u : 0u)
	                                                                       | ((w.has_contact && w.ground_dynamic) ? (w.contact_body + 1u) << 5 : 0u)));
	if (c == VEH_CHUNK_LONG) return F4(w.contact_long, w.comb_long_fric);
	if (c == VEH_CHUNK_LAT) return F4(w.contact_lat, w.comb_lat_fric);
	if (c == VEH_CHUNK_GVEL) return F4(w.contact_point_vel, w.brake_impulse);
	if (c == VEH_CHUNK_CPOS) return F4(w.contact_pos, w.angular_velocity);
	if (c == VEH_CHUNK_MISC) return make_float4(w.radius, w.inertia, w.suspension.softness, w.suspension.bias);
	if (c == VEH_CHUNK_WPOS) return F4(w.position, w.sus_min);
	if (c == VEH_CHUNK_SDIR) return F4(w.suspension_dir, w.axle_plane_constant);
	const sgd_axis_part& p = *part[(c - VEH_CHUNK_ROW) >> 1];
	return ((c - VEH_CHUNK_ROW) & 1) ? F4(p.iI_r1xa, p.lambda) : F4(p.r1xa, p.eff);
}
SGP_DEV void veh_export(const DV& d, uint32_t k, const sgd_vehicle& v, int deferred)
{
	const int i = (int)(threadIdx.x & 3u), c = (int)(threadIdx.x >> 2);
	d.veh_rows[veh_chunk_at(d, k, i, c)] = veh_export_chunk(v, i, c);
	if (threadIdx.x < VEH_HEAD_F4) {
		const uint32_t bits = (v.active ? 1u : 0u) | ((v.is_motorcycle && v.lean_enabled) ? 2u : 0u) | (deferred ? 4u : 0u);
		float4 h;
		if (threadIdx.x == 0) h = make_float4(__uint_as_float(v.body), __uint_as_float(bits), __uint_as_float((uint32_t)v.num_wheels), v.lean_integrated_delta);
		else if (threadIdx.x == 1) h = F4(v.forward, v.lean_spring_constant);
		else if (threadIdx.x == 2) h = F4(v.up, v.lean_spring_damping);
		else if (threadIdx.x == 3) h = F4(v.target_lean, v.lean_integration_coefficient);
		else h = make_float4(v.lean_integration_decay, v.lean_applied_impulse, 0.0f, 0.0f);
		d.veh_head[(size_t)k * VEH_HEAD_F4 + threadIdx.x] = h;
	}
}

struct VehBody { v3 v, w; float im; sym33 I; };
struct VehGround { uint32_t id; v3 v, w; float im; sym33 I; v3 r2; };
SGP_DEV void veh_row_solve(VehBody& c, VehGround& g, float4 ra, float4& ri, float softness, float bias, v3 ground_vel, v3 axis, float lo, float hi)
{
	const v3 r1xa = V3(ra), iI = V3(ri);
	const bool two = g.id != SGP_INVALID_ID;
	v3 r2xa = V3(0.0f, 0.0f, 0.0f), iI2 = r2xa;
	float jv;
	if (two) {
		r2xa = v3_cross(g.r2, axis);
		iI2 = sym33_mul(g.I, r2xa);
		jv = (v3_dot(axis, v3_sub(c.v, g.v)) + v3_dot(r1xa, c.w)) - v3_dot(r2xa, g.w);
	} else jv = v3_dot(axis, v3_sub(c.v, ground_vel)) + v3_dot(r1xa, c.w);
	const float lambda = ra.w * (jv - (softness * ri.w + bias));
	const float nl = clampf(ri.w + lambda, lo, hi);
	const float dl = nl - ri.w;
	c.v = v3_sub(c.v, v3_scale(axis, dl * c.im));
	c.w = v3_sub(c.w, v3_scale(iI, dl));
	if (two) {
		g.v = v3_add(g.v, v3_scale(axis, dl * g.im));
		g.w = v3_add(g.w, v3_scale(iI2, dl));
	}
	ri.w = nl;
}
SGP_DEV void veh_row_apply(VehBody& c, VehGround& g, float4 ri, v3 axis)
{
	c.v = v3_sub(c.v, v3_scale(axis, ri.w * c.im));
	c.w = v3_sub(c.w, v3_scale(V3(ri), ri.w));
	if (g.id != SGP_INVALID_ID) {
		g.v = v3_add(g.v, v3_scale(axis, ri.w * g.im));
		g.w = v3_add(g.w, v3_scale(sym33_mul(g.I, v3_cross(g.r2, axis)), ri.w));
	}
}
template <int I> SGP_DEV uint32_t quad_bcast_u(uint32_t x) { return (uint32_t)__builtin_amdgcn_mov_dpp((int)x, I * 0x55, 0xF, 0xF, true); }
#define VEH_TURN(WI, ...) { if (L == WI) { __VA_ARGS__ } c.v = quad_bcast<WI>(c.v); c.w = quad_bcast<WI>(c.w); \
	{ const uint32_t og = quad_bcast_u<WI>(g.id); const v3 ov = quad_bcast<WI>(g.v), ow = quad_bcast<WI>(g.w); if (g.id != SGP_INVALID_ID && og == g.id) { g.v = ov; g.w = ow; } } }
#define VEH_TURNS(...) VEH_TURN(0, __VA_ARGS__) VEH_TURN(1, __VA_ARGS__) VEH_TURN(2, __VA_ARGS__) VEH_TURN(3, __VA_ARGS__)

template <int MODE> SGP_DEV void veh_quad_solve(const DV& d, uint32_t k, int L, bool deferred_pass)
{
	if (k >= d.n_vehicles) return;
	const float4 h0 = d.veh_head[(size_t)k * VEH_HEAD_F4];
	const uint32_t hbits = __float_as_uint(h0.y);
	if (!(hbits & 1u)) return;
	if (((hbits & 4u) != 0u) != deferred_pass) return;
	const uint32_t b = __float_as_uint(h0.x);
	const int nw = (int)__float_as_uint(h0.z);
	sgd_vehicle* gv = &d.vehicles[k];
	sgd_wheel* gw = &gv->wheels[L];
	const float4 cn = d.veh_rows[veh_chunk_at(d, k, L, VEH_CHUNK_NORMAL)];
	const uint32_t wbits = L < nw ? __float_as_uint(cn.w) : 0u;
	const bool contact = wbits & 1u;
	const uint32_t gid = (wbits >> 5) ? (wbits >> 5) - 1u : SGP_INVALID_ID;
	const v3 neg_n = v3_neg(V3(cn));
	if (MODE == 2) {
		const float4 cp = d.veh_rows[veh_chunk_at(d, k, L, VEH_CHUNK_CPOS)], wp = d.veh_rows[veh_chunk_at(d, k, L, VEH_CHUNK_WPOS)], sd = d.veh_rows[veh_chunk_at(d, k, L, VEH_CHUNK_SDIR)];
		const float4 p4 = d.pose[POSE_F4 * (size_t)b], q4 = d.pose[POSE_F4 * (size_t)b + 1];
		const v3 iil = V3(d.pose[POSE_F4 * (size_t)b + 2]);
		v3 pos = V3(p4); quat rot = Q4(q4);
		const float im = p4.w, baumgarte = d.st.baumgarte;
		float4 gp4 = make_float4(0.0f, 0.0f, 0.0f, 0.0f), gq4 = make_float4(0.0f, 0.0f, 0.0f, 1.0f); v3 giil = V3(0.0f, 0.0f, 0.0f);
		if (gid != SGP_INVALID_ID) { gp4 = d.pose[POSE_F4 * (size_t)gid]; gq4 = d.pose[POSE_F4 * (size_t)gid + 1]; giil = V3(d.pose[POSE_F4 * (size_t)gid + 2]); }
		v3 gpos = V3(gp4); quat grot = Q4(gq4);
		bool gmoved = false;
#define VEH_POS_TURN(WI) { \
		if (L == WI && contact) { \
			const m33 R = quat_to_m33(rot); \
			const v3 ws_dir = m33_mul(R, V3(sd)); \
			const v3 ws_pos = v3_add(pos, m33_mul(R, V3(wp))); \
			const v3 min_pos = v3_add(ws_pos, v3_scale(ws_dir, wp.w)); \
			const float err = v3_dot(V3(cn), min_pos) - sd.w; \
			if (err < 0.0f) { \
				const v3 r1 = v3_sub(V3(cp), pos); \
				const sym33 I = world_inv_inertia(R, iil); \
				const v3 r1xa = v3_cross(r1, neg_n); \
				const v3 iI = sym33_mul(I, r1xa); \
				float inv_eff = im + v3_dot(r1xa, iI); \
				v3 iI2 = V3(0.0f, 0.0f, 0.0f); \
				if (gid != SGP_INVALID_ID) { \
					const v3 r2xa = v3_cross(v3_sub(V3(cp), gpos), neg_n); \
					iI2 = sym33_mul(world_inv_inertia(quat_to_m33(grot), giil), r2xa); \
					inv_eff = inv_eff + (gp4.w + v3_dot(r2xa, iI2)); \
				} \
				if (inv_eff > 0.0f) { \
					const float lambda = -(1.0f / inv_eff) * baumgarte * err; \
					pos = v3_sub(pos, v3_scale(neg_n, lambda * im)); \
					rot = quat_add_rotation_step(rot, v3_scale(iI, -lambda)); \
					if (gid != SGP_INVALID_ID) { \
						gpos = v3_add(gpos, v3_scale(neg_n, lambda * gp4.w)); \
						grot = quat_add_rotation_step(grot, v3_scale(iI2, lambda)); \
						gmoved = true; \
					} \
				} \
			} \
		} \
		pos = quad_bcast<WI>(pos); rot.x = quad_bcast<WI>(rot.x); rot.y = quad_bcast<WI>(rot.y); rot.z = quad_bcast<WI>(rot.z); rot.w = quad_bcast<WI>(rot.w); \
		{ const uint32_t og = quad_bcast_u<WI>(gid); const v3 op = quad_bcast<WI>(gpos); const float ox = quad_bcast<WI>(grot.x), oy = quad_bcast<WI>(grot.y), oz = quad_bcast<WI>(grot.z), ow = quad_bcast<WI>(grot.w); \
		  if (L != WI && gid != SGP_INVALID_ID && og == gid) { gpos = op; grot.x = ox; grot.y = oy; grot.z = oz; grot.w = ow; } } }
		VEH_POS_TURN(0) VEH_POS_TURN(1) VEH_POS_TURN(2) VEH_POS_TURN(3)
#undef VEH_POS_TURN
		if (L == 0) { d.pose[POSE_F4 * (size_t)b] = F4(pos, p4.w); d.pose[POSE_F4 * (size_t)b + 1] = make_float4(rot.x, rot.y, rot.z, rot.w); }
		if (gmoved) { d.pose[POSE_F4 * (size_t)gid] = F4(gpos, gp4.w); d.pose[POSE_F4 * (size_t)gid + 1] = make_float4(grot.x, grot.y, grot.z, grot.w); }
		return;
	}
	float4 ra[4], ri[4];
#pragma unroll
	for (int r = 0; r < 4; ++r) { ra[r] = d.veh_rows[veh_chunk_at(d, k, L, VEH_CHUNK_ROW + 2 * r)]; ri[r] = d.veh_rows[veh_chunk_at(d, k, L, VEH_CHUNK_ROW + 2 * r + 1)]; }
	const float4 s0 = d.vel[VEL_F4 * (size_t)b], s1 = d.vel[VEL_F4 * (size_t)b + 1];
	VehBody c;
	c.v = V3(s0); c.im = s0.w; c.w = V3(s1);
	const quat crot = Q4(d.pose[POSE_F4 * (size_t)b + 1]);
	c.I = c.im > 0.0f ? world_inv_inertia(quat_to_m33(crot), V3(d.pose[POSE_F4 * (size_t)b + 2])) : sym33_zero();
	float4 cp = d.veh_rows[veh_chunk_at(d, k, L, VEH_CHUNK_CPOS)];
	VehGround g; g.id = gid; g.v = V3(0.0f, 0.0f, 0.0f); g.w = g.v; g.im = 0.0f; g.I = sym33_zero(); g.r2 = g.v;
	float4 g0 = make_float4(0.0f, 0.0f, 0.0f, 0.0f), g1 = g0;
	if (gid != SGP_INVALID_ID) {
		g0 = d.vel[VEL_F4 * (size_t)gid]; g1 = d.vel[VEL_F4 * (size_t)gid + 1];
		const float4 gp4 = d.pose[POSE_F4 * (size_t)gid];
		g.v = V3(g0); g.w = V3(g1); g.im = gp4.w;
		g.I = world_inv_inertia(quat_to_m33(Q4(d.pose[POSE_F4 * (size_t)gid + 1])), V3(d.pose[POSE_F4 * (size_t)gid + 2]));
		g.r2 = v3_sub(V3(cp), V3(gp4));
	}
	if (MODE == 0) {
		const v3 neg_lat = v3_neg(V3(d.veh_rows[veh_chunk_at(d, k, L, VEH_CHUNK_LAT)]));
		VEH_TURNS(if (contact) { if (wbits & 2u) veh_row_apply(c, g, ri[0], neg_n); if (wbits & 4u) veh_row_apply(c, g, ri[1], neg_n); if (wbits & 16u) veh_row_apply(c, g, ri[3], neg_lat); })
		if (L == 0) { d.vel[VEL_F4 * (size_t)b] = F4(c.v, s0.w); d.vel[VEL_F4 * (size_t)b + 1] = F4(c.w, s1.w); }
		if (gid != SGP_INVALID_ID) { d.vel[VEL_F4 * (size_t)gid] = F4(g.v, g0.w); d.vel[VEL_F4 * (size_t)gid + 1] = F4(g.w, g1.w); }
		return;
	}
	const float4 cl = d.veh_rows[veh_chunk_at(d, k, L, VEH_CHUNK_LONG)], ct = d.veh_rows[veh_chunk_at(d, k, L, VEH_CHUNK_LAT)], cg = d.veh_rows[veh_chunk_at(d, k, L, VEH_CHUNK_GVEL)];
	const float4 cm = d.veh_rows[veh_chunk_at(d, k, L, VEH_CHUNK_MISC)];
	const v3 cpos = V3(d.pose[POSE_F4 * (size_t)b]);
	const v3 gvel = V3(cg);
	VEH_TURNS(if (contact) { if (wbits & 2u) veh_row_solve(c, g, ra[0], ri[0], cm.z, cm.w, gvel, neg_n, 0.0f, 3.0e38f); if (wbits & 4u) veh_row_solve(c, g, ra[1], ri[1], 0.0f, 0.0f, gvel, neg_n, 0.0f, 3.0e38f); })
	const float sus_lambda = ri[0].w + ri[1].w;
	const float max_long = cl.w * sus_lambda, max_lat = contact ? ct.w * sus_lambda : 0.0f;
	VEH_TURNS(if (contact && (wbits & 8u)) {
		const v3 rel = v3_sub(v3_add(c.v, v3_cross(c.w, v3_sub(V3(cp), cpos))), gvel);
		const float rel_long = v3_dot(rel, V3(cl));
		if (cg.w != 0.0f) {
			const float bi = fminf(cg.w, max_long);
			float lo, hi;
			if (rel_long >= 0.0f) { lo = -bi; hi = 0.0f; } else { lo = 0.0f; hi = bi; }
			veh_row_solve(c, g, ra[2], ri[2], 0.0f, 0.0f, gvel, v3_neg(V3(cl)), lo, hi);
		} else {
			const float desired_w = rel_long / cm.x;
			const float lin_imp = (cp.w - desired_w) * cm.y / cm.x;
			const float prev = ri[2].w;
			const float lim = clampf(prev + lin_imp, -max_long, max_long);
			veh_row_solve(c, g, ra[2], ri[2], 0.0f, 0.0f, gvel, v3_neg(V3(cl)), lim, lim);
			cp.w = cp.w - (ri[2].w - prev) * cm.x / cm.y;
		}
	})
	VEH_TURNS(if (contact && (wbits & 16u)) veh_row_solve(c, g, ra[3], ri[3], 0.0f, 0.0f, gvel, v3_neg(V3(ct)), -max_lat, max_lat);)
	float lean_integrated = h0.w, lean_applied = 0.0f;
	if (hbits & 2u) {
		const float4 h1 = d.veh_head[(size_t)k * VEH_HEAD_F4 + 1], h2 = d.veh_head[(size_t)k * VEH_HEAD_F4 + 2], h3 = d.veh_head[(size_t)k * VEH_HEAD_F4 + 3], h4 = d.veh_head[(size_t)k * VEH_HEAD_F4 + 4];
		lean_applied = h4.y;
		const float lam = ri[0].w + ri[1].w;
		const v3 arm = v3_sub(V3(cp), cpos);
		const float lam_w[4] = { quad_bcast<0>(lam), quad_bcast<1>(lam), quad_bcast<2>(lam), quad_bcast<3>(lam) };
		const v3 arm_w[4] = { quad_bcast<0>(arm), quad_bcast<1>(arm), quad_bcast<2>(arm), quad_bcast<3>(arm) };
		const uint32_t con = contact ? 1u : 0u;
		const uint32_t con_w[4] = { quad_bcast_u<0>(con), quad_bcast_u<1>(con), quad_bcast_u<2>(con), quad_bcast_u<3>(con) };
		bool all_in_contact = true;
#pragma unroll
		for (int i = 0; i < 4; ++i) if (i < nw && (!con_w[i] || !(lam_w[i] > 0.0f))) all_in_contact = false;
		const float dt = d.sp->dt;
		if (all_in_contact) {
			const m33 R = quat_to_m33(crot);
			const v3 forward = m33_mul(R, V3(h1)), up = m33_mul(R, V3(h2));
			const v3 target = V3(h3);
			const float d_angle = -sgd_signf(v3_dot(v3_cross(target, up), forward)) * sgd_acos11(clampf(v3_dot(target, up), -1.0f, 1.0f));
			const float ddt_angle = v3_dot(c.w, forward);
			const v3 If = sym33_mul(c.I, forward);
			const float iff = v3_dot(forward, If);
			const float wf0 = ddt_angle - iff * lean_applied;
			const float total = (h1.w * d_angle - h2.w * wf0 + h3.w * lean_integrated) * dt / (1.0f + h2.w * dt * iff);
			const v3 old_w = c.w;
			c.w = v3_add(c.w, v3_scale(If, total - lean_applied));
			lean_applied = total;
			const v3 dw = v3_sub(c.w, old_w);
			v3 lin_acc = V3(0.0f, 0.0f, 0.0f); float total_lambda = 0.0f;
#pragma unroll
			for (int i = 0; i < 4; ++i) if (i < nw) { total_lambda = total_lambda + lam_w[i]; lin_acc = v3_add(lin_acc, v3_scale(v3_cross(dw, arm_w[i]), lam_w[i])); }
			c.v = v3_sub(c.v, v3_scale(lin_acc, 1.0f / total_lambda));
		} else lean_integrated = lean_integrated * fmaxf(0.0f, 1.0f - h4.x * dt);
	}
	if (L < nw) {
#pragma unroll
		for (int r = 0; r < 4; ++r) d.veh_rows[veh_chunk_at(d, k, L, VEH_CHUNK_ROW + 2 * r + 1)] = ri[r];
		d.veh_rows[veh_chunk_at(d, k, L, VEH_CHUNK_CPOS)] = cp;
		gw->suspension.lambda = ri[0].w; gw->max_up.lambda = ri[1].w; gw->longitudinal.lambda = ri[2].w; gw->lateral.lambda = ri[3].w;
		gw->angular_velocity = cp.w;
	}
	if (gid != SGP_INVALID_ID) { d.vel[VEL_F4 * (size_t)gid] = F4(g.v, g0.w); d.vel[VEL_F4 * (size_t)gid + 1] = F4(g.w, g1.w); }
	if (L == 0) {
		d.vel[VEL_F4 * (size_t)b] = F4(c.v, s0.w); d.vel[VEL_F4 * (size_t)b + 1] = F4(c.w, s1.w);
		if (hbits & 2u) {
			d.veh_head[(size_t)k * VEH_HEAD_F4] = make_float4(h0.x, h0.y, h0.z, lean_integrated);
			float4* h4p = &d.veh_head[(size_t)k * VEH_HEAD_F4 + 4];
			*h4p = make_float4(h4p->x, lean_applied, 0.0f, 0.0f);
			gv->lean_integrated_delta = lean_integrated; gv->lean_applied_impulse = lean_applied;
		}
	}
}
#undef VEH_TURNS
#undef VEH_TURN

template <int MODE> SGP_DEV void veh_block_solve(const DV& d, uint32_t block, uint32_t n_blocks)
{
	__shared__ uint32_t s_veh_ticket;
	const uint32_t t = block * blockDim.x + threadIdx.x;
	veh_quad_solve<MODE>(d, t >> 2, (int)(t & 3u), false);
	if (d.ctr->veh_deferred == 0u) return;
	__syncthreads();
	if (threadIdx.x == 0) { __threadfence(); s_veh_ticket = atomicAdd(&d.ctr->veh_done, 1u); }
	__syncthreads();
	if (s_veh_ticket != n_blocks - 1u) return;
	if (threadIdx.x == 0) d.ctr->veh_done = 0u;
	__threadfence();
	if (threadIdx.x >= 4u) return;
	const uint32_t n_words = (d.n_vehicles + 31u) >> 5;
	for (uint32_t wd = 0; wd < n_words; ++wd) {
		uint32_t bits = d.veh_defer_bits[wd];
		while (bits) {
			const uint32_t k = (wd << 5) + (uint32_t)__ffs((int)bits) - 1u;
			bits &= bits - 1u;
			veh_quad_solve<MODE>(d, k, (int)threadIdx.x, true);
			__threadfence_block();
		}
	}
}

#define VEH_SOLVE_TPB SOLVE_VEL_TPB
template <int MODE> __global__ void __launch_bounds__(VEH_SOLVE_TPB) k_vehicle_solve(DV d)
{
	veh_block_solve<MODE>(d, blockIdx.x, gridDim.x);
}

template <int MODE, int ROWS = -1> __global__ void __launch_bounds__(SOLVE_VEL_TPB) k_solve_colour_veh(DV d, int colour_arg, uint32_t veh_blocks)
{
	const int colour = colour_arg & 0xFF;
	if (blockIdx.x < veh_blocks) {
		veh_block_solve<MODE>(d, blockIdx.x, veh_blocks);
		return;
	}
	const uint32_t first = d.cstarts[colour], end = d.cstarts[colour + 1];
	const int side = (int)(threadIdx.x & 1u);
	const uint32_t cb = blockIdx.x - veh_blocks, cg = gridDim.x - veh_blocks;
	const uint32_t bx = (colour_arg & SOLVE_XCD_CHUNKS) ? (cb & 7u) * (cg >> 3) + (cb >> 3) : cb;
	for (uint32_t k = first + ((bx * SOLVE_VEL_TPB + threadIdx.x) >> 1); k < end; k += cg * (SOLVE_VEL_TPB / 2)) {
		if (MODE == 1) solve_velocity_pair_t<VEL_F4, ROWS>(d, k, side, d.vel); else solve_position_pair(d, k, side);
	}
}
void launch_solve_colour_veh(const DV& d, int colour, uint32_t est, int mode, hipStream_t s, int compact_rows)
{
	uint32_t blocks = (est + est / 8 + 64 + SOLVE_VEL_TPB / 2 - 1) / (SOLVE_VEL_TPB / 2);
	if (blocks > 8192) blocks = 8192;
	blocks = (blocks + 7u) & ~7u;
	if (est >= 8192u && est <= 65536u) colour |= SOLVE_XCD_CHUNKS;
	const uint32_t vb = (d.n_vehicles * 4u + SOLVE_VEL_TPB - 1) / SOLVE_VEL_TPB;
	if (mode == 1) {
		if (compact_rows == 2) hipLaunchKernelGGL((k_solve_colour_veh<1, 2>), dim3(vb + blocks), dim3(SOLVE_VEL_TPB), 0, s, d, colour, vb);
		else if (compact_rows) hipLaunchKernelGGL((k_solve_colour_veh<1, 1>), dim3(vb + blocks), dim3(SOLVE_VEL_TPB), 0, s, d, colour, vb);
		else hipLaunchKernelGGL((k_solve_colour_veh<1, 0>), dim3(vb + blocks), dim3(SOLVE_VEL_TPB), 0, s, d, colour, vb);
	}
	else hipLaunchKernelGGL((k_solve_colour_veh<2, -1>), dim3(vb + blocks), dim3(SOLVE_VEL_TPB), 0, s, d, colour, vb);
}
void launch_vehicle_pre(const DV& d, bool cylinder_testers, hipStream_t s)
{
	if (!d.n_vehicles) return;
	if (cylinder_testers) hipLaunchKernelGGL(k_vehicle_cast<true>, dim3(d.n_vehicles), dim3(64), 0, s, d);
	else hipLaunchKernelGGL(k_vehicle_cast<false>, dim3(d.n_vehicles), dim3(64), 0, s, d);
	hipLaunchKernelGGL(k_vehicle_controller, dim3(d.n_vehicles), dim3(64), 0, s, d);
}
void launch_vehicle_solve(const DV& d, int mode, hipStream_t s)
{
	const dim3 g((d.n_vehicles * 4u + VEH_SOLVE_TPB - 1) / VEH_SOLVE_TPB), b(VEH_SOLVE_TPB);
	if (mode == 0) hipLaunchKernelGGL(k_vehicle_solve<0>, g, b, 0, s, d);
	else if (mode == 1) hipLaunchKernelGGL(k_vehicle_solve<1>, g, b, 0, s, d);
	else hipLaunchKernelGGL(k_vehicle_solve<2>, g, b, 0, s, d);
}
```

Before: 550.4 steps/s.

## Hoist constraint-array selection and issue point loads early in colour solve kernels

Resolves the parity-selected ConstraintArrays once per kernel into scalar registers, so the pointer is no longer re-derived through d.sp->parity on every access. Kernel arguments are reordered so cstarts and step params come first, and empty asm statements keep the needed pointers in scalar registers. Per-point row, lambda and location loads are issued up front, ahead of the inertia and velocity or pose loads, to overlap memory latency. This raises SGPR pressure and depends on compiler behaviour around the inline-asm hints.

After: 598.6 steps/s, median of 6. 1.09x the previous value.

```diff
diff --git a/substrata_amd/csrc/sgp_dev_common.h b/substrata_amd/csrc/sgp_dev_common.h
--- a/substrata_amd/csrc/sgp_dev_common.h
+++ b/substrata_amd/csrc/sgp_dev_common.h
@@ -10,6 +10,35 @@
 
 SGP_DEV const ConstraintArrays& CUR(const DV& d) { return d.ca[d.sp->parity & 1]; }
 SGP_DEV const ConstraintArrays& PRV(const DV& d) { return d.ca[(d.sp->parity & 1) ^ 1]; }
+SGP_DEV ConstraintArrays cur_arrays(const DV& d, uint32_t parity)
+{
+	const bool odd = (parity & 1u) != 0u;
+	const ConstraintArrays &a = d.ca[0], &b = d.ca[1];
+	const auto pick = [odd](auto pa, auto pb) { return odd ? pb : pa; };
+	ConstraintArrays c;
+	c.hdr = pick(a.hdr, b.hdr); c.n_fric = pick(a.n_fric, b.n_fric); c.prec = pick(a.prec, b.prec);
+#pragma unroll
+	for (int i = 0; i < 4; ++i) {
+		c.r1b[i] = pick(a.r1b[i], b.r1b[i]); c.r2e[i] = pick(a.r2e[i], b.r2e[i]); c.lam[i] = pick(a.lam[i], b.lam[i]);
+		c.efft[i] = pick(a.efft[i], b.efft[i]); c.loc1[i] = pick(a.loc1[i], b.loc1[i]); c.loc2[i] = pick(a.loc2[i], b.loc2[i]);
+	}
+	return c;
+}
+enum { CA_ARMS = 1, CA_LAM = 2, CA_LOC = 4 };
+#define SGP_KEEP4(a) "s"((a)[0]), "s"((a)[1]), "s"((a)[2]), "s"((a)[3])
+template <int WHAT> SGP_DEV void keep_buffer(const ConstraintArrays& c)
+{
+	if constexpr (WHAT == CA_ARMS) asm volatile("" :: "s"(c.hdr), "s"(c.n_fric), SGP_KEEP4(c.r1b), SGP_KEEP4(c.r2e), SGP_KEEP4(c.efft), SGP_KEEP4(c.lam));
+	else if constexpr (WHAT == CA_LAM) asm volatile("" :: "s"(c.hdr), "s"(c.n_fric), SGP_KEEP4(c.lam));
+	else asm volatile("" :: "s"(c.hdr), "s"(c.n_fric), SGP_KEEP4(c.loc1), SGP_KEEP4(c.loc2));
+}
+template <int WHAT> SGP_DEV void keep_head(const DV& d, uint32_t parity, uint32_t first, uint32_t end, const void* records, uint32_t grid)
+{
+	asm volatile("" :: "s"(parity), "s"(first), "s"(end), "s"(records), "s"(grid));
+	if constexpr (WHAT == CA_LAM) asm volatile("" :: "s"(d.rows), "s"(d.cap_manifolds));
+	keep_buffer<WHAT>(d.ca[0]);
+	keep_buffer<WHAT>(d.ca[1]);
+}
 SGP_DEV uint2 con_ab(const ConstraintArrays& c, size_t k) { return *(const uint2*)(c.hdr + k); }
 SGP_DEV int& con_npc(const ConstraintArrays& c, size_t k) { return ((int*)(c.hdr + k))[2]; }
 SGP_DEV uint4 con_hdr(const ConstraintArrays& c, size_t k) { return c.hdr[k]; }
diff --git a/substrata_amd/csrc/sgp_dev_solve.h b/substrata_amd/csrc/sgp_dev_solve.h
--- a/substrata_amd/csrc/sgp_dev_solve.h
+++ b/substrata_amd/csrc/sgp_dev_solve.h
@@ -15,6 +15,9 @@
 {
 	return __int_as_float(__builtin_amdgcn_mov_dpp(__float_as_int(x), 0xB1, 0xF, 0xF, true));
 }
+
+template <class F> SGP_DEV void more_points(int np, F f) { if (np > 1) { f(1); if (np > 2) { f(2); if (np > 3) f(3); } } }
+template <class F> SGP_DEV void for_points(int np, F f) { f(0); more_points(np, f); }
 
 struct ConHalf {
 	uint32_t body;
@@ -27,7 +30,7 @@
 	v3     lam[4];
 };
 
-template <int ROWS = -1> SGP_DEV void half_load_rows(const DV& d, uint32_t slot, int side, ConHalf& h)
+template <int ROWS = -1> SGP_DEV void half_load_rows(const DV& d, const ConstraintArrays& ca, uint32_t slot, int side, ConHalf& h)
 {
 	const int np = h.np_col & 0xFF;
 	const size_t st = d.cap_manifolds;
@@ -36,19 +39,18 @@
 		const v3 n = V3(h.nf);
 		h.t1 = v3_normalized_perpendicular(n);
 		const v3 t2 = v3_cross(n, h.t1);
+		float4 r4[4]; float2 et[4];
+		for_points(np, [&](int i) { r4[i] = (side ? ca.r2e[i] : ca.r1b[i])[slot]; et[i] = ca.efft[i][slot]; h.lam[i] = V3(ca.lam[i][slot]); });
 #pragma unroll
 		for (int i = 0; i < 4; ++i) {
 			if (i == 0 || i < np) {
-				const float4 r4 = side ? CUR(d).r2e[i][slot] : CUR(d).r1b[i][slot];
-				const float2 et = CUR(d).efft[i][slot];
-				const v3 r = V3(r4);
+				const v3 r = V3(r4[i]);
 				h.c[i][0] = v3_cross(r, n); h.c[i][1] = v3_cross(r, h.t1); h.c[i][2] = v3_cross(r, t2);
 #pragma unroll
 				for (int a = 0; a < 3; ++a) h.iv[i][a] = sym33_mul(I, h.c[i][a]);
-				const float ow = lane_swap1(r4.w);
-				h.eff[i][0] = side ? r4.w : ow; h.bias[i] = side ? ow : r4.w;
-				h.eff[i][1] = et.x; h.eff[i][2] = et.y;
-				h.lam[i] = V3(CUR(d).lam[i][slot]);
+				const float ow = lane_swap1(r4[i].w);
+				h.eff[i][0] = side ? r4[i].w : ow; h.bias[i] = side ? ow : r4[i].w;
+				h.eff[i][1] = et[i].x; h.eff[i][2] = et[i].y;
 			}
 		}
 		return;
@@ -66,7 +68,7 @@
 					h.eff[i][a] = side ? c4.w : ow;
 					if (a == 0) h.bias[i] = side ? ow : c4.w;
 				}
-				h.lam[i] = V3(CUR(d).lam[i][slot]);
+				h.lam[i] = V3(ca.lam[i][slot]);
 			}
 		}
 		h.t1 = v3_normalized_perpendicular(V3(h.nf));
@@ -89,32 +91,35 @@
 					if (a == 0) { h.t1.x = side ? oi : i4.w; h.t1.y = side ? i4.w : oi; } else h.t1.z = side ? oi : i4.w;
 				}
 			}
-			const float4 l4 = CUR(d).lam[i][slot];
+			const float4 l4 = ca.lam[i][slot];
 			h.lam[i] = V3(l4);
 		}
 	}
 }
 
-template <int ROWS = -1> SGP_DEV void half_load_known(const DV& d, uint32_t slot, int side, int np_col, uint32_t body, ConHalf& h)
+template <int ROWS = -1> SGP_DEV void half_load_known(const DV& d, const ConstraintArrays& ca, uint32_t slot, int side, int np_col, uint32_t body, ConHalf& h)
 {
 	h.body = body;
-	h.nf = CUR(d).n_fric[slot];
+	h.nf = ca.n_fric[slot];
 	h.np_col = np_col;
-	half_load_rows<ROWS>(d, slot, side, h);
-}
-template <int ROWS = -1> SGP_DEV void half_load(const DV& d, uint32_t slot, int side, ConHalf& h)
-{
-	const uint4 hd = con_hdr(CUR(d), slot);
-	half_load_known<ROWS>(d, slot, side, (int)hd.z, side ? hd.y : hd.x, h);
-}
-
-SGP_DEV void half_store(const DV& d, uint32_t slot, int side, const ConHalf& h)
+	half_load_rows<ROWS>(d, ca, slot, side, h);
+}
+template <int ROWS = -1> SGP_DEV void half_load(const DV& d, const ConstraintArrays& ca, uint32_t slot, int side, ConHalf& h)
+{
+	const uint4 hd = con_hdr(ca, slot);
+	half_load_known<ROWS>(d, ca, slot, side, (int)hd.z, side ? hd.y : hd.x, h);
+}
+
+SGP_DEV void half_store(const ConstraintArrays& ca, uint32_t slot, int side, const ConHalf& h)
 {
 	if (side) return;
 	const int np = h.np_col & 0xFF;
 #pragma unroll
-	for (int i = 0; i < 4; ++i) { if (i < np) CUR(d).lam[i][slot] = F4(h.lam[i], 0.0f); }
-}
+	for (int i = 0; i < 4; ++i) { if (i < np) ca.lam[i][slot] = F4(h.lam[i], 0.0f); }
+}
+
+template <int ROWS = -1> SGP_DEV void half_load(const DV& d, uint32_t slot, int side, ConHalf& h) { half_load<ROWS>(d, CUR(d), slot, side, h); }
+SGP_DEV void half_store(const DV& d, uint32_t slot, int side, const ConHalf& h) { half_store(CUR(d), slot, side, h); }
 
 SGP_DEV float half_jv(v3 lv, v3 av, v3 axis, v3 c, int side)
 {
@@ -171,37 +176,34 @@
 	if (half_solve_core(h, side, v4, w4, dbg)) { vel[VS * (size_t)h.body] = v4; vel[VS * (size_t)h.body + 1] = w4; }
 }
 
-template <int VS, int ROWS = -1> SGP_DEV void solve_velocity_pair_t(const DV& d, uint32_t slot, int side, float4* vel)
+template <int VS, int ROWS = -1> SGP_DEV void solve_velocity_pair_t(const DV& d, const ConstraintArrays& ca, uint32_t slot, int side, float4* vel)
 {
 	ConHalf h;
-	half_load<ROWS>(d, slot, side, h);
+	half_load<ROWS>(d, ca, slot, side, h);
 	half_solve<VS>(h, side, vel, d.dbg_flags);
-	half_store(d, slot, side, h);
-}
-
-template <int VS> SGP_DEV void solve_velocity_pair_norows(const DV& d, uint32_t slot, int side, float4* vel)
-{
-	const uint4 hd = con_hdr(CUR(d), slot);
+	half_store(ca, slot, side, h);
+}
+
+template <int VS, int ROWS = -1> SGP_DEV void solve_velocity_pair_t(const DV& d, uint32_t slot, int side, float4* vel) { solve_velocity_pair_t<VS, ROWS>(d, CUR(d), slot, side, vel); }
+
+template <int VS> SGP_DEV void solve_velocity_pair_norows(const DV& d, const ConstraintArrays& ca, uint32_t slot, int side, float4* vel)
+{
+	const uint4 hd = con_hdr(ca, slot);
 	const int np = (int)hd.z & 0xFF;
 	const uint32_t body = side ? hd.y : hd.x;
-	const float4 nf = CUR(d).n_fric[slot];
+	const float4 nf = ca.n_fric[slot];
 	float4 r4[4]; float2 et[4]; v3 lam[4];
-#pragma unroll
-	for (int i = 0; i < 4; ++i) {
-		if (i == 0 || i < np) { r4[i] = side ? CUR(d).r2e[i][slot] : CUR(d).r1b[i][slot]; et[i] = CUR(d).efft[i][slot]; lam[i] = V3(CUR(d).lam[i][slot]); }
-		else { r4[i] = make_float4(0.0f, 0.0f, 0.0f, 0.0f); et[i] = make_float2(0.0f, 0.0f); lam[i] = V3(0.0f, 0.0f, 0.0f); }
-	}
-	if (np == 0) return;
+	const auto load_point = [&](int i) { r4[i] = (side ? ca.r2e[i] : ca.r1b[i])[slot]; et[i] = ca.efft[i][slot]; lam[i] = V3(ca.lam[i][slot]); };
+	load_point(0);
 	const sym33 I = body_world_inv_inertia_rec(d, body);
 	float4 v4 = vel[VS * (size_t)body], w4 = vel[VS * (size_t)body + 1];
+	more_points(np, load_point);
+	if (np == 0) return;
 	const float im = v4.w, friction = nf.w;
 	v3 lv = V3(v4), av = V3(w4);
 	const v3 n = V3(nf);
 	const v3 t1 = v3_normalized_perpendicular(n);
 	const v3 t2 = v3_cross(n, t1);
-	float eff0[4], bias[4];
-#pragma unroll
-	for (int i = 0; i < 4; ++i) { const float ow = lane_swap1(r4[i].w); eff0[i] = side ? r4[i].w : ow; bias[i] = side ? ow : r4[i].w; }
 	if (friction > 0.0f) {
 #pragma unroll
 		for (int i = 0; i < 4; ++i) {
@@ -220,10 +222,13 @@
 	}
 #pragma unroll
 	for (int i = 0; i < 4; ++i) {
-		if (i < np && eff0[i] > 0.0f) {
+		if (i >= np) continue;
+		const float ow = lane_swap1(r4[i].w);
+		const float eff0 = side ? r4[i].w : ow, bias = side ? ow : r4[i].w;
+		if (eff0 > 0.0f) {
 			const v3 c0 = v3_cross(V3(r4[i]), n);
 			const float jv = half_jv(lv, av, n, c0, side);
-			const float lambda = eff0[i] * (jv - bias[i]);
+			const float lambda = eff0 * (jv - bias);
 			const float nl = max0f(lam[i].x + lambda);
 			half_apply(lv, av, im, n, sym33_mul(I, c0), nl - lam[i].x, side);
 			lam[i].x = nl;
@@ -232,25 +237,23 @@
 	if (im > 0.0f) { vel[VS * (size_t)body] = F4(lv, im); vel[VS * (size_t)body + 1] = F4(av, 0.0f); }
 	if (!side) {
 #pragma unroll
-		for (int i = 0; i < 4; ++i) { if (i < np) CUR(d).lam[i][slot] = F4(lam[i], 0.0f); }
+		for (int i = 0; i < 4; ++i) { if (i < np) ca.lam[i][slot] = F4(lam[i], 0.0f); }
 	}
 }
 
 struct PosHalf { float4 nf; int np; v3 loc[4]; };
-SGP_DEV void pos_half_load(const DV& d, uint32_t slot, int side, int np_col, PosHalf& ph)
-{
-	ph.nf = CUR(d).n_fric[slot];
+SGP_DEV void pos_half_load(const ConstraintArrays& ca, uint32_t slot, int side, int np_col, PosHalf& ph)
+{
+	ph.nf = ca.n_fric[slot];
 	ph.np = np_col & 0xFF;
-#pragma unroll
-	for (int i = 0; i < 4; ++i) if (i == 0 || i < ph.np) ph.loc[i] = V3(side ? CUR(d).loc2[i][slot] : CUR(d).loc1[i][slot]);
-}
-SGP_DEV void pos_half_solve(const DV& d, const PosHalf& ph, int side, float4* rec, v3 ii)
+	for_points(ph.np, [&](int i) { ph.loc[i] = V3((side ? ca.loc2[i] : ca.loc1[i])[slot]); });
+}
+SGP_DEV void pos_half_solve_rec(const DV& d, const PosHalf& ph, int side, float4* rec, float4 p4, float4 q4, v3 ii)
 {
 	const v3 nrm = V3(ph.nf);
 	const int np = ph.np;
-	const float4 p4 = rec[0];
 	const float im = p4.w;
-	quat q = Q4(rec[1]);
+	quat q = Q4(q4);
 	v3 pos = V3(p4);
 	bool moved = false;
 	m33 R = quat_to_m33(q);
@@ -284,18 +287,25 @@
 	}
 	if (moved && im > 0.0f) { rec[0] = F4(pos, im); rec[1] = make_float4(q.x, q.y, q.z, q.w); }
 }
-SGP_DEV void solve_position_pair(const DV& d, uint32_t slot, int side)
-{
-	const uint4 hd = con_hdr(CUR(d), slot);
+SGP_DEV void pos_half_solve(const DV& d, const PosHalf& ph, int side, float4* rec, v3 ii) { pos_half_solve_rec(d, ph, side, rec, rec[0], rec[1], ii); }
+SGP_DEV void solve_position_pair(const DV& d, const ConstraintArrays& ca, uint32_t slot, int side)
+{
+	const uint4 hd = con_hdr(ca, slot);
 	const uint32_t body = side ? hd.y : hd.x;
 	PosHalf ph;
-	pos_half_load(d, slot, side, (int)hd.z, ph);
-	pos_half_solve(d, ph, side, d.pose + POSE_F4 * (size_t)body, V3(d.pose[POSE_F4 * (size_t)body + 2]));
-}
-SGP_DEV void solve_position_pair_at(const DV& d, uint32_t slot, int side, float4* rec, v3 ii)
+	ph.nf = ca.n_fric[slot];
+	ph.np = (int)hd.z & 0xFF;
+	const auto load_point = [&](int i) { ph.loc[i] = V3((side ? ca.loc2[i] : ca.loc1[i])[slot]); };
+	load_point(0);
+	float4* rec = d.pose + POSE_F4 * (size_t)body;
+	const float4 p4 = rec[0], q4 = rec[1], i4 = rec[2];
+	more_points(ph.np, load_point);
+	pos_half_solve_rec(d, ph, side, rec, p4, q4, V3(i4));
+}
+SGP_DEV void solve_position_pair_at(const DV& d, const ConstraintArrays& ca, uint32_t slot, int side, float4* rec, v3 ii)
 {
 	PosHalf ph;
-	pos_half_load(d, slot, side, con_npc(CUR(d), slot), ph);
+	pos_half_load(ca, slot, side, con_npc(ca, slot), ph);
 	pos_half_solve(d, ph, side, rec, ii);
 }
 #define SOLVE_VEL_TPB 256
diff --git a/substrata_amd/csrc/sgp_k_solve.hip b/substrata_amd/csrc/sgp_k_solve.hip
--- a/substrata_amd/csrc/sgp_k_solve.hip
+++ b/substrata_amd/csrc/sgp_k_solve.hip
@@ -21,11 +21,11 @@
 }
 
 struct PairCtx { uint2 ab; float im1, im2; sym33 I1, I2; BodyVel A, B; v3 n, t1, t2; float friction; int np; };
-template <int VS> SGP_DEV void load_pair(const DV& d, uint32_t slot, PairCtx& c, const float4* vel)
-{
-	const uint4 hd = con_hdr(CUR(d), slot);
+template <int VS> SGP_DEV void load_pair(const DV& d, const ConstraintArrays& ca, uint32_t slot, PairCtx& c, const float4* vel)
+{
+	const uint4 hd = con_hdr(ca, slot);
 	c.ab = make_uint2(hd.x, hd.y);
-	const float4 nf = CUR(d).n_fric[slot];
+	const float4 nf = ca.n_fric[slot];
 	c.n = V3(nf); c.friction = nf.w;
 	c.np = (int)hd.z & 0xFF;
 	const float4 va = vel[VS * (size_t)c.ab.x], wa = vel[VS * (size_t)c.ab.x + 1];
@@ -37,24 +37,26 @@
 	c.B.lv = V3(vb); c.B.av = V3(wb);
 }
 
+template <int VS> SGP_DEV void load_pair(const DV& d, uint32_t slot, PairCtx& c, const float4* vel) { load_pair<VS>(d, CUR(d), slot, c, vel); }
+
 template <int VS> SGP_DEV void store_pair_vel(const PairCtx& c, float4* vel)
 {
 	if (c.im1 > 0.0f) { vel[VS * (size_t)c.ab.x] = F4(c.A.lv, c.im1); vel[VS * (size_t)c.ab.x + 1] = F4(c.A.av, 0.0f); }
 	if (c.im2 > 0.0f) { vel[VS * (size_t)c.ab.y] = F4(c.B.lv, c.im2); vel[VS * (size_t)c.ab.y + 1] = F4(c.B.av, 0.0f); }
 }
 
-template <int VS> SGP_DEV void warm_start_one_t(const DV& d, uint32_t slot, float4* vel)
+template <int VS> SGP_DEV void warm_start_one_t(const DV& d, const ConstraintArrays& ca, uint32_t slot, float4* vel)
 {
 	PairCtx c;
-	load_pair<VS>(d, slot, c, vel);
+	load_pair<VS>(d, ca, slot, c, vel);
 	c.t1 = v3_normalized_perpendicular(c.n);
 	c.t2 = v3_cross(c.n, c.t1);
 	v3 P = V3(0.0f, 0.0f, 0.0f), A1 = V3(0.0f, 0.0f, 0.0f), A2 = V3(0.0f, 0.0f, 0.0f);
 #pragma unroll
 	for (int i = 0; i < 4; ++i) {
 		if (i < c.np) {
-			const v3 r1 = V3(CUR(d).r1b[i][slot]), r2 = V3(CUR(d).r2e[i][slot]);
-			const float4 l = CUR(d).lam[i][slot];
+			const v3 r1 = V3(ca.r1b[i][slot]), r2 = V3(ca.r2e[i][slot]);
+			const float4 l = ca.lam[i][slot];
 			v3 j = v3_scale(c.n, l.x);
 			if (c.friction > 0.0f) { j = v3_add(j, v3_scale(c.t1, l.y)); j = v3_add(j, v3_scale(c.t2, l.z)); }
 			P = v3_add(P, j);
@@ -66,7 +68,7 @@
 	if (c.im2 > 0.0f) { c.B.lv = v3_add(c.B.lv, v3_scale(P, c.im2)); c.B.av = v3_add(c.B.av, sym33_mul(c.I2, A2)); }
 	store_pair_vel<VS>(c, vel);
 }
-SGP_DEV void warm_start_one(const DV& d, uint32_t slot) { warm_start_one_t<VEL_F4>(d, slot, d.vel); }
+SGP_DEV void warm_start_one(const DV& d, const ConstraintArrays& ca, uint32_t slot) { warm_start_one_t<VEL_F4>(d, ca, slot, d.vel); }
 
 SGP_DEV void warm_body_one(const DV& d, uint32_t i)
 {
@@ -93,16 +95,16 @@
 	rec[0] = F4(lv, im);
 	rec[1] = F4(av, 0.0f);
 }
-SGP_DEV void warm_start_one(const DV& d, uint32_t k);
-SGP_DEV uint32_t overflow_next(const DV& d, uint32_t first, uint32_t count, uint64_t& last, bool& have_last);
+SGP_DEV uint32_t overflow_next(const ConstraintArrays& ca, uint32_t first, uint32_t count, uint64_t& last, bool& have_last);
 __global__ void __launch_bounds__(TPB) k_warm_bodies(DV d)
 {
 	warm_body_one(d, blockIdx.x * TPB + threadIdx.x);
 	const uint32_t first = d.cstarts[SGP_OVERFLOW_COLOUR], count = d.cstarts[SGP_OVERFLOW_COLOUR + 1] - first;
 	if (count == 0u) return;
 	if (!last_block(&d.ctr->tickets[1]) || threadIdx.x != 0) return;
+	const ConstraintArrays ca = cur_arrays(d, d.sp->parity);
 	uint64_t last = 0; bool have_last = false;
-	for (uint32_t it = 0; it < count; ++it) warm_start_one(d, overflow_next(d, first, count, last, have_last));
+	for (uint32_t it = 0; it < count; ++it) warm_start_one(d, ca, overflow_next(ca, first, count, last, have_last));
 }
 struct AxisRows { float4 c1, c2, i1, i2; };
 
@@ -131,11 +133,11 @@
 	}
 }
 
-SGP_DEV void solve_position_one(const DV& d, uint32_t slot)
-{
-	const uint4 hd = con_hdr(CUR(d), slot);
+SGP_DEV void solve_position_one(const DV& d, const ConstraintArrays& ca, uint32_t slot)
+{
+	const uint4 hd = con_hdr(ca, slot);
 	const uint2 ab = make_uint2(hd.x, hd.y);
-	const float4 nf = CUR(d).n_fric[slot];
+	const float4 nf = ca.n_fric[slot];
 	const v3 nrm = V3(nf);
 	const int np = (int)hd.z & 0xFF;
 	float4* ra = d.pose + POSE_F4 * (size_t)ab.x;
@@ -150,8 +152,8 @@
 #pragma unroll
 	for (int i = 0; i < 4; ++i) {
 		if (i >= np) continue;
-		const v3 p1 = v3_add(posA, m33_mul(RA, V3(CUR(d).loc1[i][slot])));
-		const v3 p2 = v3_add(posB, m33_mul(RB, V3(CUR(d).loc2[i][slot])));
+		const v3 p1 = v3_add(posA, m33_mul(RA, V3(ca.loc1[i][slot])));
+		const v3 p2 = v3_add(posB, m33_mul(RB, V3(ca.loc2[i][slot])));
 		float sep = v3_dot(v3_sub(p2, p1), nrm) + d.st.penetration_slop;
 		if (sep < 0.0f) {
 			sep = fmaxf(sep, -d.st.max_penetration_distance);
@@ -183,38 +185,43 @@
 }
 
 #define SOLVE_TPB 64
-template <int MODE, int ROWS = -1, int OCC = 1> __global__ void __launch_bounds__(MODE != 0 ? SOLVE_VEL_TPB : SOLVE_TPB, OCC) k_solve_colour(const uint32_t* cstarts_pre, StepParams* sp_pre, DV d_arg, int colour_arg)
+template <int MODE, int ROWS = -1, int OCC = 1> __global__ void __launch_bounds__(MODE != 0 ? SOLVE_VEL_TPB : SOLVE_TPB, OCC) k_solve_colour(const uint32_t* cstarts_pre, StepParams* sp_pre, int colour_arg, DV d_arg)
 {
 	DV d = d_arg; d.sp = sp_pre;
 	const int colour = colour_arg & 0xFF;
+	const uint32_t parity = sp_pre->parity;
 	const uint32_t first = cstarts_pre[colour], end = cstarts_pre[colour + 1];
+	keep_head<MODE == 2 ? CA_LOC : (MODE == 0 || ROWS == 2) ? CA_ARMS : CA_LAM>(d_arg, parity, first, end, MODE == 2 ? d_arg.pose : d_arg.vel, gridDim.x);
+	const ConstraintArrays ca = cur_arrays(d_arg, parity);
 	if (MODE != 0) {
 		const int side = (int)(threadIdx.x & 1u);
 		const uint32_t bx = (colour_arg & SOLVE_XCD_CHUNKS) ? xcd_block() : blockIdx.x;
 		for (uint32_t k = first + ((bx * SOLVE_VEL_TPB + threadIdx.x) >> 1); k < end; k += gridDim.x * (SOLVE_VEL_TPB / 2)) {
-			if (MODE == 1) { if constexpr (ROWS == 2) solve_velocity_pair_norows<VEL_F4>(d, k, side, d.vel); else solve_velocity_pair_t<VEL_F4, ROWS>(d, k, side, d.vel); }
-			else solve_position_pair(d, k, side);
+			if (MODE == 1) { if constexpr (ROWS == 2) solve_velocity_pair_norows<VEL_F4>(d, ca, k, side, d.vel); else solve_velocity_pair_t<VEL_F4, ROWS>(d, ca, k, side, d.vel); }
+			else solve_position_pair(d, ca, k, side);
 		}
 		return;
 	}
-	for (uint32_t k = first + blockIdx.x * SOLVE_TPB + threadIdx.x; k < end; k += gridDim.x * SOLVE_TPB) warm_start_one(d, k);
-}
-
-
-SGP_DEV uint32_t overflow_next(const DV& d, uint32_t first, uint32_t count, uint64_t& last, bool& have_last)
+	for (uint32_t k = first + blockIdx.x * SOLVE_TPB + threadIdx.x; k < end; k += gridDim.x * SOLVE_TPB) warm_start_one(d, ca, k);
+}
+
+
+SGP_DEV uint32_t overflow_next(const ConstraintArrays& ca, uint32_t first, uint32_t count, uint64_t& last, bool& have_last)
 {
 	uint64_t best = ~0ull; uint32_t bslot = first;
 	for (uint32_t k = 0; k < count; ++k) {
-		const uint2 okab = con_ab(CUR(d), first + k); const uint64_t pr = sgp_mix64(((uint64_t)okab.x << 32) | okab.y);
+		const uint2 okab = con_ab(ca, first + k); const uint64_t pr = sgp_mix64(((uint64_t)okab.x << 32) | okab.y);
 		if ((!have_last || pr > last) && pr <= best) { best = pr; bslot = first + k; }
 	}
 	last = best; have_last = true;
 	return bslot;
 }
+SGP_DEV uint32_t overflow_next(const DV& d, uint32_t first, uint32_t count, uint64_t& last, bool& have_last) { return overflow_next(CUR(d), first, count, last, have_last); }
 
 __global__ void __launch_bounds__(512) k_solve_tail(DV d, int first_colour, int mode)
 {
 	__shared__ uint32_t cs[SGP_MAX_COLOURS + 1];
+	const ConstraintArrays ca = cur_arrays(d, d.sp->parity);
 	if (threadIdx.x <= SGP_MAX_COLOURS) cs[threadIdx.x] = d.cstarts[threadIdx.x];
 	__syncthreads();
 	if (cs[first_colour] == cs[SGP_MAX_COLOURS]) return;
@@ -222,7 +229,7 @@
 		const uint32_t b = cs[c], e = cs[c + 1];
 		if (b == e) continue;
 		for (uint32_t k = b + threadIdx.x; k < e; k += 512) {
-			if (mode == 0) warm_start_one(d, k); else solve_position_one(d, k);
+			if (mode == 0) warm_start_one(d, ca, k); else solve_position_one(d, ca, k);
 		}
 		__syncthreads();
 	}
@@ -230,8 +237,8 @@
 	if (count == 0 || threadIdx.x != 0) return;
 	uint64_t last = 0; bool have_last = false;
 	for (uint32_t it = 0; it < count; ++it) {
-		const uint32_t bslot = overflow_next(d, first, count, last, have_last);
-		if (mode == 0) warm_start_one(d, bslot); else solve_position_one(d, bslot);
+		const uint32_t bslot = overflow_next(ca, first, count, last, have_last);
+		if (mode == 0) warm_start_one(d, ca, bslot); else solve_position_one(d, ca, bslot);
 	}
 }
 
@@ -239,6 +246,7 @@
 template <int ROWS> __global__ void __launch_bounds__(TAIL_VEL_TPB) k_solve_tail_vel(DV d, int first_colour)
 {
 	__shared__ uint32_t cs[SGP_MAX_COLOURS + 1];
+	const ConstraintArrays ca = cur_arrays(d, d.sp->parity);
 	if (threadIdx.x <= SGP_MAX_COLOURS) cs[threadIdx.x] = d.cstarts[threadIdx.x];
 	__syncthreads();
 	if (cs[first_colour] == cs[SGP_MAX_COLOURS]) return;
@@ -249,26 +257,26 @@
 		const uint32_t slot = cs[first_colour] + pair;
 		const bool mine = pair < tail_n;
 		ConHalf h; int my_col = -1;
-		if (mine) { half_load<ROWS>(d, slot, side, h); my_col = (h.np_col >> 8) & 0xFF; }
+		if (mine) { half_load<ROWS>(d, ca, slot, side, h); my_col = (h.np_col >> 8) & 0xFF; }
 		for (int c = first_colour; c < SGP_OVERFLOW_COLOUR; ++c) {
 			if (cs[c] == cs[c + 1]) continue;
 			if (my_col == c) half_solve<VEL_F4>(h, side, d.vel, d.dbg_flags);
 			__syncthreads();
 		}
-		if (mine) half_store(d, slot, side, h);
+		if (mine) half_store(ca, slot, side, h);
 	} else
 	for (int c = first_colour; c < SGP_OVERFLOW_COLOUR; ++c) {
 		const uint32_t b = cs[c], e = cs[c + 1];
 		if (b == e) continue;
-		for (uint32_t k = b + pair; k < e; k += TAIL_VEL_TPB / 2) solve_velocity_pair_t<VEL_F4, ROWS>(d, k, side, d.vel);
+		for (uint32_t k = b + pair; k < e; k += TAIL_VEL_TPB / 2) solve_velocity_pair_t<VEL_F4, ROWS>(d, ca, k, side, d.vel);
 		__syncthreads();
 	}
 	const uint32_t first = cs[SGP_OVERFLOW_COLOUR], count = cs[SGP_OVERFLOW_COLOUR + 1] - first;
 	if (count == 0 || threadIdx.x >= 2) return;
 	uint64_t last = 0; bool have_last = false;
 	for (uint32_t it = 0; it < count; ++it) {
-		const uint32_t bslot = overflow_next(d, first, count, last, have_last);
-		solve_velocity_pair_t<VEL_F4, ROWS>(d, bslot, side, d.vel);
+		const uint32_t bslot = overflow_next(ca, first, count, last, have_last);
+		solve_velocity_pair_t<VEL_F4, ROWS>(d, ca, bslot, side, d.vel);
 	}
 }
 #define HC_CLASSES 9
@@ -283,12 +291,13 @@
 
 __global__ void __launch_bounds__(TPB) k_hc_hook(DV d, int first_colour)
 {
+	const ConstraintArrays ca = cur_arrays(d, d.sp->parity);
 	const uint32_t b = d.cstarts[first_colour], e = d.cstarts[SGP_OVERFLOW_COLOUR];
 	const uint32_t tid = blockIdx.x * TPB + threadIdx.x, stride = gridDim.x * TPB;
 	const uint32_t lim = min(2u * (e - b) + HC_CLASSES * HC_WG_PAIRS, d.cap_hc_list);
 	for (uint32_t i = tid; i < lim; i += stride) d.hc_list[i] = HC_NONE;
 	for (uint32_t k = b + tid; k < e; k += stride) {
-		const uint2 ab = con_ab(CUR(d), k);
+		const uint2 ab = con_ab(ca, k);
 		if (!hc_can_move(d, ab.x) || !hc_can_move(d, ab.y)) continue;
 		uint32_t ra = uf_find(d.hc_root, ab.x), rb = uf_find(d.hc_root, ab.y);
 		while (ra != rb) {
@@ -307,20 +316,22 @@
 }
 __global__ void __launch_bounds__(TPB) k_hc_count(DV d, int first_colour)
 {
+	const ConstraintArrays ca = cur_arrays(d, d.sp->parity);
 	const uint32_t b = d.cstarts[first_colour], e = d.cstarts[SGP_OVERFLOW_COLOUR];
 	for (uint32_t k = b + blockIdx.x * TPB + threadIdx.x; k < e; k += gridDim.x * TPB) {
-		const uint32_t r = hc_root_of(d, con_ab(CUR(d), k));
+		const uint32_t r = hc_root_of(d, con_ab(ca, k));
 		d.hc_rank[k] = r == HC_NONE ? 0u : atomicAdd(&d.hc_count[r], 1u);
 	}
 }
 __global__ void __launch_bounds__(TPB) k_hc_alloc(DV d, int first_colour)
 {
+	const ConstraintArrays ca = cur_arrays(d, d.sp->parity);
 	const uint32_t b = d.cstarts[first_colour], e = d.cstarts[SGP_OVERFLOW_COLOUR];
 	const int lane = (int)(threadIdx.x & 63u);
 	for (uint32_t k0 = b + blockIdx.x * TPB; k0 < e; k0 += gridDim.x * TPB) {
 		const uint32_t k = k0 + threadIdx.x;
 		uint32_t r = HC_NONE, size = 0;
-		if (k < e && d.hc_rank[k] == 0u) { r = hc_root_of(d, con_ab(CUR(d), k)); if (r != HC_NONE) size = d.hc_count[r]; }
+		if (k < e && d.hc_rank[k] == 0u) { r = hc_root_of(d, con_ab(ca, k)); if (r != HC_NONE) size = d.hc_count[r]; }
 		const bool lead = r != HC_NONE;
 		int cls = -1;
 		if (lead) {
@@ -345,10 +356,11 @@
 }
 __global__ void __launch_bounds__(TPB) k_hc_scatter(DV d, int first_colour)
 {
+	const ConstraintArrays ca = cur_arrays(d, d.sp->parity);
 	const uint32_t b = d.cstarts[first_colour], e = d.cstarts[SGP_OVERFLOW_COLOUR];
 	if (blockIdx.x == 0 && threadIdx.x == 0) { d.ctr->hc_entries = hc_class_first(d, HC_CLASSES); d.ctr->hc_n = e - b; }
 	for (uint32_t k = b + blockIdx.x * TPB + threadIdx.x; k < e; k += gridDim.x * TPB) {
-		const uint32_t r = hc_root_of(d, con_ab(CUR(d), k));
+		const uint32_t r = hc_root_of(d, con_ab(ca, k));
 		const uint32_t place = r == HC_NONE ? HC_BIG : d.hc_base[r];
 		uint32_t at = HC_NONE;
 		if (place != HC_BIG) {
@@ -357,7 +369,7 @@
 		}
 		if (at < d.cap_hc_list) d.hc_list[at] = k;
 		else {
-			con_npc(CUR(d), k) |= NPCOL_CATCH_ALL;
+			con_npc(ca, k) |= NPCOL_CATCH_ALL;
 			const uint32_t bi = wave_alloc(&d.ctr->hc_n_big);
 			if (bi < HC_BIG_LIST) d.hc_big_list[bi] = k;
 		}
@@ -366,19 +378,21 @@
 
 __global__ void __launch_bounds__(TPB) k_hc_init(DV d, int first_colour)
 {
+	const ConstraintArrays ca = cur_arrays(d, d.sp->parity);
 	const uint32_t b = d.cstarts[first_colour], e = d.cstarts[SGP_OVERFLOW_COLOUR];
 	for (uint32_t k = b + blockIdx.x * TPB + threadIdx.x; k < e; k += gridDim.x * TPB) {
-		const uint2 ab = con_ab(CUR(d), k);
+		const uint2 ab = con_ab(ca, k);
 		if (hc_can_move(d, ab.x)) { d.hc_root[ab.x] = ab.x; d.hc_count[ab.x] = 0u; }
 		if (hc_can_move(d, ab.y)) { d.hc_root[ab.y] = ab.y; d.hc_count[ab.y] = 0u; }
 	}
 }
 __global__ void __launch_bounds__(TPB) k_hc_probe(DV d, int first_colour)
 {
+	const ConstraintArrays ca = cur_arrays(d, d.sp->parity);
 	const uint32_t b = d.cstarts[first_colour], e = d.cstarts[SGP_OVERFLOW_COLOUR];
 	for (uint32_t k = b + blockIdx.x * TPB + threadIdx.x; k < e; k += gridDim.x * TPB) {
 		if (d.hc_rank[k] != 0u) continue;
-		const uint32_t r = hc_root_of(d, con_ab(CUR(d), k));
+		const uint32_t r = hc_root_of(d, con_ab(ca, k));
 		if (r == HC_NONE) continue;
 		const uint32_t size = d.hc_count[r];
 		if (size > (uint32_t)HC_WG_PAIRS) atomicAdd(&d.ctr->hc_probe_big, size);
@@ -387,6 +401,7 @@
 
 __global__ void __launch_bounds__(HC_WG_PAIRS) k_hc_sort(DV d)
 {
+	const ConstraintArrays ca = cur_arrays(d, d.sp->parity);
 	__shared__ uint32_t s_cnt[SGP_MAX_COLOURS], s_first[SGP_MAX_COLOURS];
 	__shared__ uint4 s_slot[HC_WG_PAIRS];
 	const uint32_t entries = d.ctr->hc_entries;
@@ -394,7 +409,7 @@
 		if (threadIdx.x < SGP_MAX_COLOURS) s_cnt[threadIdx.x] = 0u;
 		__syncthreads();
 		const uint32_t slot = d.hc_list[e0 + threadIdx.x];
-		const uint4 hd = slot != HC_NONE ? con_hdr(CUR(d), slot) : make_uint4(0u, 0u, 0u, 0u);
+		const uint4 hd = slot != HC_NONE ? con_hdr(ca, slot) : make_uint4(0u, 0u, 0u, 0u);
 		const int npc = (int)hd.z;
 		const uint2 ab = make_uint2(hd.x, hd.y);
 		const int col = slot != HC_NONE ? ((npc >> 8) & 0xFF) : SGP_MAX_COLOURS - 1;
@@ -415,7 +430,7 @@
 }
 
 #define HC_TABLE 1024
-template <int MODE, int ROWS = -1> __global__ void __launch_bounds__(HC_TPB) k_solve_hc(const StepCounters* ctr_pre, const uint4* hc_entry_pre, DV d, int first_colour)
+template <int MODE, int ROWS = -1> __global__ void __launch_bounds__(HC_TPB) k_solve_hc(const StepCounters* ctr_pre, const uint4* hc_entry_pre, const StepParams* sp_pre, int first_colour, DV d)
 {
 	constexpr int RS = MODE == 1 ? 2 : 3;
 	__shared__ float4 s_rec[HC_TABLE * RS];
@@ -424,8 +439,14 @@
 	__shared__ uint32_t s_ticket;
 	const int side = (int)(threadIdx.x & 1u);
 	const uint32_t pair = threadIdx.x >> 1;
+	const uint32_t parity = sp_pre->parity;
 	const uint32_t entries = ctr_pre->hc_entries;
 	const int n_colours = (int)ctr_pre->n_colours;
+	constexpr bool RESOLVE = MODE == 2 || ROWS == 2;
+	if constexpr (RESOLVE) keep_head<MODE == 2 ? CA_LOC : CA_ARMS>(d, parity, entries, (uint32_t)n_colours, MODE == 2 ? d.pose : d.vel, gridDim.x);
+	ConstraintArrays resolved;
+	if constexpr (RESOLVE) resolved = cur_arrays(d, parity);
+	const auto ca = [&]() -> const ConstraintArrays& { if constexpr (RESOLVE) return resolved; else return CUR(d); };
 	for (uint32_t e0 = blockIdx.x * HC_WG_PAIRS; e0 < entries; e0 += gridDim.x * HC_WG_PAIRS) {
 		__syncthreads();
 		for (uint32_t i = threadIdx.x; i < HC_TABLE; i += HC_TPB) s_key[i] = HC_NONE;
@@ -439,7 +460,7 @@
 		if (mine) {
 			my_col = ((int)entry.y >> 8) & 0xFF;
 			body = side ? entry.w : entry.z;
-			if (MODE == 1) half_load_known<ROWS>(d, slot, side, (int)entry.y, body, h); else pos_half_load(d, slot, side, (int)entry.y, ph);
+			if (MODE == 1) half_load_known<ROWS>(d, ca(), slot, side, (int)entry.y, body, h); else pos_half_load(ca(), slot, side, (int)entry.y, ph);
 			if (side == 0) atomicOr(&s_present, 1ull << my_col);
 			at = uf_prio(body) & (HC_TABLE - 1);
 			for (;;) {
@@ -462,7 +483,7 @@
 			if (my_col == c) { if (MODE == 1) half_solve<2>(h, side, s_rec, d.dbg_flags); else pos_half_solve(d, ph, side, s_rec + RS * at, V3(s_rec[RS * at + 2])); }
 			__syncthreads();
 		}
-		if (MODE == 1 && mine) half_store(d, slot, side, h);
+		if (MODE == 1 && mine) half_store(ca(), slot, side, h);
 		if (owner && s_rec[RS * at].w > 0.0f) {
 			float4* g = (MODE == 1 ? d.vel + VEL_F4 * (size_t)body : d.pose + POSE_F4 * (size_t)body);
 			g[0] = s_rec[RS * at]; g[1] = s_rec[RS * at + 1];
@@ -482,7 +503,7 @@
 		for (uint32_t e = pair; e < n_big; e += HC_WG_PAIRS) { const uint32_t k = d.hc_big_list[e]; mine[cnt] = k; mcol[cnt] = (int)((con_npc(CUR(d), k) >> 8) & 0xFF); ++cnt; }
 		for (int c = first_colour; c < n_colours; ++c) {
 #pragma unroll
-			for (int j = 0; j < 4; ++j) if (j < cnt && mcol[j] == c) { if (MODE == 1) solve_velocity_pair_t<VEL_F4, ROWS>(d, mine[j], side, d.vel); else solve_position_pair(d, mine[j], side); }
+			for (int j = 0; j < 4; ++j) if (j < cnt && mcol[j] == c) { if (MODE == 1) solve_velocity_pair_t<VEL_F4, ROWS>(d, CUR(d), mine[j], side, d.vel); else solve_position_pair(d, CUR(d), mine[j], side); }
 			__syncthreads();
 		}
 	} else
@@ -490,15 +511,15 @@
 		const uint32_t cb = d.cstarts[c], ce = d.cstarts[c + 1];
 		for (uint32_t k = cb + pair; k < ce; k += HC_WG_PAIRS) {
 			if (!(con_npc(CUR(d), k) & NPCOL_CATCH_ALL)) continue;
-			if (MODE == 1) solve_velocity_pair_t<VEL_F4, ROWS>(d, k, side, d.vel); else solve_position_pair(d, k, side);
+			if (MODE == 1) solve_velocity_pair_t<VEL_F4, ROWS>(d, CUR(d), k, side, d.vel); else solve_position_pair(d, CUR(d), k, side);
 		}
 		__syncthreads();
 	}
 	if (ocount == 0u || threadIdx.x >= 2u) return;
 	uint64_t last = 0; bool have_last = false;
 	for (uint32_t it = 0; it < ocount; ++it) {
-		const uint32_t bslot = overflow_next(d, ofirst, ocount, last, have_last);
-		if (MODE == 1) solve_velocity_pair_t<VEL_F4, ROWS>(d, bslot, side, d.vel); else solve_position_pair(d, bslot, side);
+		const uint32_t bslot = overflow_next(CUR(d), ofirst, ocount, last, have_last);
+		if (MODE == 1) solve_velocity_pair_t<VEL_F4, ROWS>(d, CUR(d), bslot, side, d.vel); else solve_position_pair(d, CUR(d), bslot, side);
 	}
 }
 
@@ -508,6 +529,7 @@
 {
 	__shared__ float4 sv[2 * SMALL_LDS_BODIES];
 	__shared__ uint32_t cs[SGP_MAX_COLOURS + 1];
+	const ConstraintArrays ca = cur_arrays(d, d.sp->parity);
 	const uint32_t n = min(d.sp->n_slots, (uint32_t)SMALL_LDS_BODIES);
 	if (threadIdx.x <= SGP_MAX_COLOURS) cs[threadIdx.x] = d.cstarts[threadIdx.x];
 	for (uint32_t i = threadIdx.x; i < 2 * n; i += SMALL_TPB) sv[i] = d.vel[VEL_F4 * (size_t)(i >> 1) + (i & 1u)];
@@ -522,12 +544,12 @@
 			for (int c = 0; c < SGP_OVERFLOW_COLOUR; ++c) {
 				const uint32_t b = cs[c], e = cs[c + 1];
 				if (b == e) continue;
-				if (side == 0 && slot >= b && slot < e) warm_start_one_t<2>(d, slot, sv);
+				if (side == 0 && slot >= b && slot < e) warm_start_one_t<2>(d, ca, slot, sv);
 				__syncthreads();
 			}
 		}
 		ConHalf h; int my_col = -1;
-		if (mine) { half_load<0>(d, slot, side, h); my_col = (h.np_col >> 8) & 0xFF; }
+		if (mine) { half_load<0>(d, ca, slot, side, h); my_col = (h.np_col >> 8) & 0xFF; }
 		for (int pass = 0; pass < iterations; ++pass) {
 			for (int c = 0; c < SGP_OVERFLOW_COLOUR; ++c) {
 				if (cs[c] == cs[c + 1]) continue;
@@ -535,15 +557,15 @@
 				__syncthreads();
 			}
 		}
-		if (mine) half_store(d, slot, side, h);
+		if (mine) half_store(ca, slot, side, h);
 	} else
 	if (cs[0] != cs[SGP_MAX_COLOURS]) {
 		for (int pass = warm_start ? -1 : 0; pass < iterations; ++pass) {
 			for (int c = 0; c < SGP_OVERFLOW_COLOUR; ++c) {
 				const uint32_t b = cs[c], e = cs[c + 1];
 				if (b == e) continue;
-				if (pass < 0) { for (uint32_t k = b + threadIdx.x; k < e; k += SMALL_TPB) warm_start_one_t<2>(d, k, sv); }
-				else { for (uint32_t k = b + pair; k < e; k += SMALL_TPB / 2) solve_velocity_pair_t<2, 0>(d, k, side, sv); }
+				if (pass < 0) { for (uint32_t k = b + threadIdx.x; k < e; k += SMALL_TPB) warm_start_one_t<2>(d, ca, k, sv); }
+				else { for (uint32_t k = b + pair; k < e; k += SMALL_TPB / 2) solve_velocity_pair_t<2, 0>(d, ca, k, side, sv); }
 				__syncthreads();
 			}
 			const uint32_t first = cs[SGP_OVERFLOW_COLOUR], count = cs[SGP_OVERFLOW_COLOUR + 1] - first;
@@ -551,8 +573,8 @@
 				if (threadIdx.x < 2) {
 					uint64_t last = 0; bool have_last = false;
 					for (uint32_t it = 0; it < count; ++it) {
-						const uint32_t bslot = overflow_next(d, first, count, last, have_last);
-						if (pass < 0) { if (side == 0) warm_start_one_t<2>(d, bslot, sv); } else solve_velocity_pair_t<2, 0>(d, bslot, side, sv);
+						const uint32_t bslot = overflow_next(ca, first, count, last, have_last);
+						if (pass < 0) { if (side == 0) warm_start_one_t<2>(d, ca, bslot, sv); } else solve_velocity_pair_t<2, 0>(d, ca, bslot, side, sv);
 					}
 				}
 				__syncthreads();
@@ -564,27 +586,27 @@
 
 struct ConReg { uint2 ab; float4 nf; int np_col; AxisRows rn[4], rt1[4], rt2[4]; float4 lam[4]; };
 
-SGP_DEV void con_load(const DV& d, uint32_t slot, ConReg& r)
-{
-	const uint4 hd = con_hdr(CUR(d), slot);
+SGP_DEV void con_load(const DV& d, const ConstraintArrays& ca, uint32_t slot, ConReg& r)
+{
+	const uint4 hd = con_hdr(ca, slot);
 	r.ab = make_uint2(hd.x, hd.y);
-	r.nf = CUR(d).n_fric[slot];
+	r.nf = ca.n_fric[slot];
 	r.np_col = (int)hd.z;
 	const int np = r.np_col & 0xFF;
 #pragma unroll
 	for (int i = 0; i < 4; ++i) {
 		if (i < np) {
 			r.rn[i] = load_axis_rows(d, slot, i, 0); r.rt1[i] = load_axis_rows(d, slot, i, 1); r.rt2[i] = load_axis_rows(d, slot, i, 2);
-			r.lam[i] = CUR(d).lam[i][slot];
-		}
-	}
-}
-
-SGP_DEV void con_store(const DV& d, uint32_t slot, const ConReg& r)
+			r.lam[i] = ca.lam[i][slot];
+		}
+	}
+}
+
+SGP_DEV void con_store(const ConstraintArrays& ca, uint32_t slot, const ConReg& r)
 {
 	const int np = r.np_col & 0xFF;
 #pragma unroll
-	for (int i = 0; i < 4; ++i) { if (i < np) CUR(d).lam[i][slot] = r.lam[i]; }
+	for (int i = 0; i < 4; ++i) { if (i < np) ca.lam[i][slot] = r.lam[i]; }
 }
 
 template <int VS> SGP_DEV void con_solve_velocity(ConReg& r, float4* vel, uint32_t dbg = 0)
@@ -628,12 +650,12 @@
 	if (im2 > 0.0f) { vel[VS * (size_t)ab.y] = F4(B.lv, im2); vel[VS * (size_t)ab.y + 1] = F4(B.av, 0.0f); }
 }
 
-template <int VS> SGP_DEV void solve_velocity_one_t(const DV& d, uint32_t slot, float4* vel)
+template <int VS> SGP_DEV void solve_velocity_one_t(const DV& d, const ConstraintArrays& ca, uint32_t slot, float4* vel)
 {
 	ConReg r;
-	con_load(d, slot, r);
+	con_load(d, ca, slot, r);
 	con_solve_velocity<VS>(r, vel, d.dbg_flags);
-	con_store(d, slot, r);
+	con_store(ca, slot, r);
 }
 __global__ void __launch_bounds__(512) k_solve_small_single(DV d, int warm_start, int iterations)
 {
@@ -651,12 +673,12 @@
 			for (int c = 0; c < SGP_OVERFLOW_COLOUR; ++c) {
 				const uint32_t b = cs[c], e = cs[c + 1];
 				if (b == e) continue;
-				if (slot >= b && slot < e) warm_start_one_t<2>(d, slot, sv);
+				if (slot >= b && slot < e) warm_start_one_t<2>(d, CUR(d), slot, sv);
 				__syncthreads();
 			}
 		}
 		ConReg r; int my_col = -1;
-		if (mine) { con_load(d, slot, r); my_col = (r.np_col >> 8) & 0xFF; }
+		if (mine) { con_load(d, CUR(d), slot, r); my_col = (r.np_col >> 8) & 0xFF; }
 		for (int pass = 0; pass < iterations; ++pass) {
 			for (int c = 0; c < SGP_OVERFLOW_COLOUR; ++c) {
 				if (cs[c] == cs[c + 1]) continue;
@@ -664,7 +686,7 @@
 				__syncthreads();
 			}
 		}
-		if (mine) con_store(d, slot, r);
+		if (mine) con_store(CUR(d), slot, r);
 	} else
 	if (cs[0] != cs[SGP_MAX_COLOURS]) {
 		for (int pass = warm_start ? -1 : 0; pass < iterations; ++pass) {
@@ -672,7 +694,7 @@
 				const uint32_t b = cs[c], e = cs[c + 1];
 				if (b == e) continue;
 				for (uint32_t k = b + threadIdx.x; k < e; k += 512) {
-					if (pass < 0) warm_start_one_t<2>(d, k, sv); else solve_velocity_one_t<2>(d, k, sv);
+					if (pass < 0) warm_start_one_t<2>(d, CUR(d), k, sv); else solve_velocity_one_t<2>(d, CUR(d), k, sv);
 				}
 				__syncthreads();
 			}
@@ -687,7 +709,7 @@
 							if ((!have_last || pr > last) && pr <= best) { best = pr; bslot = first + k; }
 						}
 						last = best; have_last = true;
-						if (pass < 0) warm_start_one_t<2>(d, bslot, sv); else solve_velocity_one_t<2>(d, bslot, sv);
+						if (pass < 0) warm_start_one_t<2>(d, CUR(d), bslot, sv); else solve_velocity_one_t<2>(d, CUR(d), bslot, sv);
 					}
 				}
 				__syncthreads();
@@ -714,15 +736,15 @@
 	if (blocks > 8192) blocks = 8192;
 	if (mode != 0) blocks = (blocks + 7u) & ~7u;
 	if (mode != 0 && est >= 8192u && est <= 65536u) colour |= SOLVE_XCD_CHUNKS;
-	if (mode == 0) hipLaunchKernelGGL(k_solve_colour<0>, dim3(blocks), dim3(SOLVE_TPB), 0, s, (const uint32_t*)d.cstarts, d.sp, d, colour);
+	if (mode == 0) hipLaunchKernelGGL(k_solve_colour<0>, dim3(blocks), dim3(SOLVE_TPB), 0, s, (const uint32_t*)d.cstarts, d.sp, colour, d);
 	else if (mode == 1) {
 		const bool many = est > SOLVE_MANY_MIN;
-		if (compact_rows == 2) hipLaunchKernelGGL((k_solve_colour<1, 2>), dim3(blocks), dim3(SOLVE_VEL_TPB), 0, s, (const uint32_t*)d.cstarts, d.sp, d, colour);
-		else if (compact_rows) { if (many) hipLaunchKernelGGL((k_solve_colour<1, 1, SOLVE_MANY_OCC>), dim3(blocks), dim3(SOLVE_VEL_TPB), 0, s, (const uint32_t*)d.cstarts, d.sp, d, colour); else hipLaunchKernelGGL((k_solve_colour<1, 1>), dim3(blocks), dim3(SOLVE_VEL_TPB), 0, s, (const uint32_t*)d.cstarts, d.sp, d, colour); }
-		else hipLaunchKernelGGL((k_solve_colour<1, 0>), dim3(blocks), dim3(SOLVE_VEL_TPB), 0, s, (const uint32_t*)d.cstarts, d.sp, d, colour);
-	}
-	else if (est > SOLVE_MANY_MIN) hipLaunchKernelGGL((k_solve_colour<2, -1, SOLVE_MANY_OCC>), dim3(blocks), dim3(SOLVE_VEL_TPB), 0, s, (const uint32_t*)d.cstarts, d.sp, d, colour);
-	else hipLaunchKernelGGL(k_solve_colour<2>, dim3(blocks), dim3(SOLVE_VEL_TPB), 0, s, (const uint32_t*)d.cstarts, d.sp, d, colour);
+		if (compact_rows == 2) hipLaunchKernelGGL((k_solve_colour<1, 2>), dim3(blocks), dim3(SOLVE_VEL_TPB), 0, s, (const uint32_t*)d.cstarts, d.sp, colour, d);
+		else if (compact_rows) { if (many) hipLaunchKernelGGL((k_solve_colour<1, 1, SOLVE_MANY_OCC>), dim3(blocks), dim3(SOLVE_VEL_TPB), 0, s, (const uint32_t*)d.cstarts, d.sp, colour, d); else hipLaunchKernelGGL((k_solve_colour<1, 1>), dim3(blocks), dim3(SOLVE_VEL_TPB), 0, s, (const uint32_t*)d.cstarts, d.sp, colour, d); }
+		else hipLaunchKernelGGL((k_solve_colour<1, 0>), dim3(blocks), dim3(SOLVE_VEL_TPB), 0, s, (const uint32_t*)d.cstarts, d.sp, colour, d);
+	}
+	else if (est > SOLVE_MANY_MIN) hipLaunchKernelGGL((k_solve_colour<2, -1, SOLVE_MANY_OCC>), dim3(blocks), dim3(SOLVE_VEL_TPB), 0, s, (const uint32_t*)d.cstarts, d.sp, colour, d);
+	else hipLaunchKernelGGL(k_solve_colour<2>, dim3(blocks), dim3(SOLVE_VEL_TPB), 0, s, (const uint32_t*)d.cstarts, d.sp, colour, d);
 }
 void launch_warm_bodies(const DV& d, uint32_t nb, hipStream_t s) { hipLaunchKernelGGL(k_warm_bodies, dim3(blocks_for(nb)), dim3(TPB), 0, s, d); }
 void launch_solve_tail(const DV& d, int first_colour, int mode, hipStream_t s, int compact_rows)
@@ -755,11 +777,11 @@
 {
 	const uint32_t blocks = std::max(1u, std::min(2048u, (2u * est + HC_CLASSES * HC_WG_PAIRS) / HC_WG_PAIRS));
 	if (mode == 1) {
-		if (compact_rows == 2) hipLaunchKernelGGL((k_solve_hc<1, 2>), dim3(blocks), dim3(HC_TPB), 0, s, (const StepCounters*)d.ctr, (const uint4*)d.hc_entry, d, first_colour);
-		else if (compact_rows) hipLaunchKernelGGL((k_solve_hc<1, 1>), dim3(blocks), dim3(HC_TPB), 0, s, (const StepCounters*)d.ctr, (const uint4*)d.hc_entry, d, first_colour);
-		else hipLaunchKernelGGL((k_solve_hc<1, 0>), dim3(blocks), dim3(HC_TPB), 0, s, (const StepCounters*)d.ctr, (const uint4*)d.hc_entry, d, first_colour);
-	}
-	else hipLaunchKernelGGL((k_solve_hc<2, -1>), dim3(blocks), dim3(HC_TPB), 0, s, (const StepCounters*)d.ctr, (const uint4*)d.hc_entry, d, first_colour);
+		if (compact_rows == 2) hipLaunchKernelGGL((k_solve_hc<1, 2>), dim3(blocks), dim3(HC_TPB), 0, s, (const StepCounters*)d.ctr, (const uint4*)d.hc_entry, (const StepParams*)d.sp, first_colour, d);
+		else if (compact_rows) hipLaunchKernelGGL((k_solve_hc<1, 1>), dim3(blocks), dim3(HC_TPB), 0, s, (const StepCounters*)d.ctr, (const uint4*)d.hc_entry, (const StepParams*)d.sp, first_colour, d);
+		else hipLaunchKernelGGL((k_solve_hc<1, 0>), dim3(blocks), dim3(HC_TPB), 0, s, (const StepCounters*)d.ctr, (const uint4*)d.hc_entry, (const StepParams*)d.sp, first_colour, d);
+	}
+	else hipLaunchKernelGGL((k_solve_hc<2, -1>), dim3(blocks), dim3(HC_TPB), 0, s, (const StepCounters*)d.ctr, (const uint4*)d.hc_entry, (const StepParams*)d.sp, first_colour, d);
 }
 void launch_solve_small(const DV& d, int warm_start, int iterations, int lane_pairs, hipStream_t s)
 {
diff --git a/substrata_amd/csrc/sgp_k_vehicle.hip b/substrata_amd/csrc/sgp_k_vehicle.hip
--- a/substrata_amd/csrc/sgp_k_vehicle.hip
+++ b/substrata_amd/csrc/sgp_k_vehicle.hip
@@ -452,19 +452,22 @@
 	veh_block_solve<MODE>(d, blockIdx.x, gridDim.x);
 }
 
-template <int MODE, int ROWS = -1> __global__ void __launch_bounds__(SOLVE_VEL_TPB) k_solve_colour_veh(DV d, int colour_arg, uint32_t veh_blocks)
+template <int MODE, int ROWS = -1> __global__ void __launch_bounds__(SOLVE_VEL_TPB) k_solve_colour_veh(const uint32_t* cstarts_pre, const StepParams* sp_pre, int colour_arg, uint32_t veh_blocks, DV d)
 {
 	const int colour = colour_arg & 0xFF;
 	if (blockIdx.x < veh_blocks) {
 		veh_block_solve<MODE>(d, blockIdx.x, veh_blocks);
 		return;
 	}
-	const uint32_t first = d.cstarts[colour], end = d.cstarts[colour + 1];
+	const uint32_t parity = sp_pre->parity;
+	const uint32_t first = cstarts_pre[colour], end = cstarts_pre[colour + 1];
+	keep_head<MODE == 2 ? CA_LOC : ROWS == 2 ? CA_ARMS : CA_LAM>(d, parity, first, end, MODE == 2 ? d.pose : d.vel, gridDim.x);
+	const ConstraintArrays ca = cur_arrays(d, parity);
 	const int side = (int)(threadIdx.x & 1u);
 	const uint32_t cb = blockIdx.x - veh_blocks, cg = gridDim.x - veh_blocks;
 	const uint32_t bx = (colour_arg & SOLVE_XCD_CHUNKS) ? (cb & 7u) * (cg >> 3) + (cb >> 3) : cb;
 	for (uint32_t k = first + ((bx * SOLVE_VEL_TPB + threadIdx.x) >> 1); k < end; k += cg * (SOLVE_VEL_TPB / 2)) {
-		if (MODE == 1) solve_velocity_pair_t<VEL_F4, ROWS>(d, k, side, d.vel); else solve_position_pair(d, k, side);
+		if (MODE == 1) solve_velocity_pair_t<VEL_F4, ROWS>(d, ca, k, side, d.vel); else solve_position_pair(d, ca, k, side);
 	}
 }
 void launch_solve_colour_veh(const DV& d, int colour, uint32_t est, int mode, hipStream_t s, int compact_rows)
@@ -475,11 +478,11 @@
 	if (est >= 8192u && est <= 65536u) colour |= SOLVE_XCD_CHUNKS;
 	const uint32_t vb = (d.n_vehicles * 4u + SOLVE_VEL_TPB - 1) / SOLVE_VEL_TPB;
 	if (mode == 1) {
-		if (compact_rows == 2) hipLaunchKernelGGL((k_solve_colour_veh<1, 2>), dim3(vb + blocks), dim3(SOLVE_VEL_TPB), 0, s, d, colour, vb);
-		else if (compact_rows) hipLaunchKernelGGL((k_solve_colour_veh<1, 1>), dim3(vb + blocks), dim3(SOLVE_VEL_TPB), 0, s, d, colour, vb);
-		else hipLaunchKernelGGL((k_solve_colour_veh<1, 0>), dim3(vb + blocks), dim3(SOLVE_VEL_TPB), 0, s, d, colour, vb);
-	}
-	else hipLaunchKernelGGL((k_solve_colour_veh<2, -1>), dim3(vb + blocks), dim3(SOLVE_VEL_TPB), 0, s, d, colour, vb);
+		if (compact_rows == 2) hipLaunchKernelGGL((k_solve_colour_veh<1, 2>), dim3(vb + blocks), dim3(SOLVE_VEL_TPB), 0, s, (const uint32_t*)d.cstarts, (const StepParams*)d.sp, colour, vb, d);
+		else if (compact_rows) hipLaunchKernelGGL((k_solve_colour_veh<1, 1>), dim3(vb + blocks), dim3(SOLVE_VEL_TPB), 0, s, (const uint32_t*)d.cstarts, (const StepParams*)d.sp, colour, vb, d);
+		else hipLaunchKernelGGL((k_solve_colour_veh<1, 0>), dim3(vb + blocks), dim3(SOLVE_VEL_TPB), 0, s, (const uint32_t*)d.cstarts, (const StepParams*)d.sp, colour, vb, d);
+	}
+	else hipLaunchKernelGGL((k_solve_colour_veh<2, -1>), dim3(vb + blocks), dim3(SOLVE_VEL_TPB), 0, s, (const uint32_t*)d.cstarts, (const StepParams*)d.sp, colour, vb, d);
 }
 void launch_vehicle_pre(const DV& d, bool cylinder_testers, hipStream_t s)
 {
```
